# google/speedy

Measured on AMD Instinct MI355X. Metric: Msamples/s processed (16 kHz mono, 3.5x nonlinear), higher is better.
Workload: dtype int16 samples; f64 DFT, f32 features, int32 AMDF/OLA

## Files before the change

### include/speedy_hip.h

```cpp
#ifndef SPEEDY_HIP_H_
#define SPEEDY_HIP_H_
#include <stddef.h>
#include <stdint.h>
#ifdef __cplusplus
extern "C" {
#endif

#ifndef SPX_FEATURE_COUNT
#define SPX_FEATURE_COUNT 15
#endif

typedef struct spx_plan* spx_plan_t;

typedef struct {
  int64_t in_off;
  int64_t n_in;
  int64_t out_off;
  int64_t out_cap;
  int32_t channels;
  float speed;
  float nonlinear;
  float feedback;
} spx_stream_job;

typedef struct {
  float* tension;
  float* speed;
  float* features;
  float* spectrogram;
  float* normalized;
} spx_taps;

const char* spx_last_error(void);
int spx_abi_version(void);

spx_plan_t spx_plan_create(int sample_rate, int match_matlab);
void spx_plan_destroy(spx_plan_t plan);
int spx_plan_frame_step(spx_plan_t plan);
int spx_plan_window_size(spx_plan_t plan);
int spx_plan_fft_size(spx_plan_t plan);
int spx_plan_future(spx_plan_t plan);
int spx_plan_max_required(spx_plan_t plan);
int64_t spx_plan_frames(spx_plan_t plan, int64_t n_in);
int64_t spx_plan_out_capacity(spx_plan_t plan, int64_t n_in, float speed);
int64_t spx_plan_out_capacity_for(spx_plan_t plan, int64_t n_in, float speed, float nonlinear);

size_t spx_batch_workspace_bytes(spx_plan_t plan, const spx_stream_job* jobs, int n_streams);

int spx_batch_run(spx_plan_t plan, const spx_stream_job* jobs, int n_streams, const int16_t* in,
                  int16_t* out, int64_t* n_out, void* workspace, size_t workspace_bytes,
                  const spx_taps* taps, void* hip_stream);

int spx_batch_run_rate(spx_plan_t plan, const spx_stream_job* jobs, const float* rates, int n_streams, const int16_t* in,
                       int16_t* out, int64_t* n_out, void* workspace, size_t workspace_bytes,
                       const spx_taps* taps, void* hip_stream);
size_t spx_batch_workspace_bytes_rate(spx_plan_t plan, const spx_stream_job* jobs, const float* rates, int n_streams);
int64_t spx_plan_out_capacity_rate(spx_plan_t plan, int64_t n_in, float speed, float nonlinear, float rate);

size_t spx_batch_workspace_bytes_float(spx_plan_t plan, const spx_stream_job* jobs, const float* rates, int n_streams);
int spx_batch_run_float(spx_plan_t plan, const spx_stream_job* jobs, const float* rates, int n_streams, const float* in,
                        float* out, int64_t* n_out, void* workspace, size_t workspace_bytes,
                        const spx_taps* taps, void* hip_stream);
int spx_float_to_short(const float* in, int16_t* out, size_t n, int nonlinear_scale, void* hip_stream);
int spx_short_to_float(const int16_t* in, float* out, size_t n, void* hip_stream);

int spx_batch_run_ahead(spx_plan_t plan, const spx_stream_job* jobs, int n_streams, const int16_t* in,
                        int16_t* out, int64_t* n_out, void* workspace, size_t workspace_bytes,
                        const spx_taps* taps, void* hip_stream);

int spx_batch_run_overlapped(spx_plan_t plan, const spx_stream_job* jobs, int n_streams, const int16_t* in,
                             int16_t* out, int64_t* n_out, void* workspace, size_t workspace_bytes,
                             const spx_taps* taps, void* hip_stream);

int spx_batch_run_ahead_when(spx_plan_t plan, const spx_stream_job* jobs, int n_streams, const int16_t* in,
                             int16_t* out, int64_t* n_out, void* workspace, size_t workspace_bytes,
                             const spx_taps* taps, void* hip_stream, void* in_ready_event);

typedef struct spx_pipeline* spx_pipeline_t;
#define SPX_PIPELINE_DEVICE_OUT 1u
#define SPX_PIPELINE_FLOAT 2u
spx_pipeline_t spx_pipeline_create(spx_plan_t plan, const spx_stream_job* jobs, int n_streams, int depth, unsigned flags);
spx_pipeline_t spx_pipeline_create_mixed(const spx_plan_t* plans, int n_plans, const spx_stream_job* jobs, const int* plan_index,
                                         int n_streams, int depth, unsigned flags);
void spx_pipeline_destroy(spx_pipeline_t p);
int spx_pipeline_depth(spx_pipeline_t p);
size_t spx_pipeline_input_values(spx_pipeline_t p);
int16_t* spx_pipeline_host_input(spx_pipeline_t p);
int64_t spx_pipeline_submit(spx_pipeline_t p, const int16_t* in, int in_is_device);
int64_t spx_pipeline_submit_jobs(spx_pipeline_t p, const spx_stream_job* jobs, const int16_t* in, int in_is_device);
int spx_pipeline_jobs_fit(spx_pipeline_t p, const spx_stream_job* jobs);
int spx_pipeline_input_consumed(spx_pipeline_t p, int64_t ticket);
int spx_pipeline_wait(spx_pipeline_t p, int64_t ticket, const int16_t** out, const int64_t** offsets, const int64_t** counts);

float* spx_pipeline_host_input_float(spx_pipeline_t p);
int64_t spx_pipeline_submit_float(spx_pipeline_t p, const float* in, int in_is_device);
int64_t spx_pipeline_submit_jobs_float(spx_pipeline_t p, const spx_stream_job* jobs, const float* in, int in_is_device);
int spx_pipeline_wait_float(spx_pipeline_t p, int64_t ticket, const float** out, const int64_t** offsets, const int64_t** counts);

void* spx_host_alloc(size_t bytes);
void spx_host_free(void* p);

int spx_batch_analyze(spx_plan_t plan, const spx_stream_job* jobs, int n_streams, const int16_t* in,
                      void* workspace, size_t workspace_bytes, const spx_taps* taps, void* hip_stream);
int spx_batch_walk(spx_plan_t plan, const spx_stream_job* jobs, int n_streams, const int16_t* in,
                   int16_t* out, int64_t* n_out, void* workspace, size_t workspace_bytes,
                   const spx_taps* taps, void* hip_stream);

size_t spx_batch_workspace_bytes_mixed(const spx_plan_t* plans, int n_plans, const spx_stream_job* jobs,
                                       const int* plan_index, int n_streams);
int spx_batch_run_mixed(const spx_plan_t* plans, int n_plans, const spx_stream_job* jobs, const int* plan_index,
                        int n_streams, const int16_t* in, int16_t* out, int64_t* n_out, void* workspace,
                        size_t workspace_bytes, void* hip_stream);

int spx_batch_run_mixed_taps(const spx_plan_t* plans, int n_plans, const spx_stream_job* jobs, const int* plan_index,
                             int n_streams, const int16_t* in, int16_t* out, int64_t* n_out, void* workspace,
                             size_t workspace_bytes, const spx_taps* taps, void* hip_stream);
int spx_batch_run_mixed_ahead(const spx_plan_t* plans, int n_plans, const spx_stream_job* jobs, const int* plan_index,
                              int n_streams, const int16_t* in, int16_t* out, int64_t* n_out, void* workspace,
                              size_t workspace_bytes, void* hip_stream);

void spx_set_timing(int enabled);
void spx_set_pipeline_chunks(int chunks);
void spx_set_concurrent(int on);
int spx_timing_collect(double* sum_ms_analyze, double* sum_ms_walk, int* n_calls);
const char* spx_batch_kernel_names(spx_plan_t plan, int n_streams, int max_channels, int speedup_only);
const char* spx_batch_kernel_names_lean(spx_plan_t plan, int n_streams, int max_channels, int speedup_only);
int spx_debug_last_walk_form(void);
int spx_debug_kernel_vgprs(int which);
int spx_debug_walk_info(int sample_rate, int channels, int n_streams, int speedup_only, int short_jobs, int lean, int* out5);
int spx_debug_analysis_info(int sample_rate, int* out4);
int spx_debug_lane_consts(int sample_rate, void* out, double* tw, double* tw2, float* win);
int spx_debug_mode_resources(int sample_rate, int channels, int n_streams, int speedup_only, long long* out22);
long long spx_debug_fdiv_check(unsigned seed, unsigned denominators, int exp_lo, int exp_hi);
long long spx_debug_xfade_check(int n_lo, int n_hi);
long long spx_debug_arith_check(unsigned seed, unsigned threads, unsigned per_thread);
int spx_debug_select_check(const unsigned* d, int n_vectors, int p0, int n_lags, int max_period, int two_per_lane, int* lag_index,
                           unsigned* kmin);
int spx_debug_select_fold_check(const unsigned* d, int n_vectors, int p0, int n_lags, int want_max, int fresh, int* out3);
int spx_debug_log_check(unsigned first_block, unsigned end_block, unsigned long long* sums);
int spx_debug_last_call_concurrent(void);
double spx_timing_last_tension_ms(void);
double spx_timing_last_rate_ms(void);

int spx_batch_read_steps(spx_plan_t plan, const spx_stream_job* jobs, int n_streams, const void* workspace,
                         int32_t* steps, void* hip_stream);
int spx_batch_read_steps_mixed(const spx_plan_t* plans, int n_plans, const spx_stream_job* jobs, const int* plan_index,
                               int n_streams, const void* workspace, int32_t* steps, void* hip_stream);

void* spx_device_alloc(size_t bytes);
void spx_device_free(void* p);
int spx_batch_pack_outputs(const spx_stream_job* jobs, int n_streams, const int16_t* out, const int64_t* n_out,
                           int16_t* packed, int64_t* offsets, void* hip_stream);
int spx_copy_to_device(void* dst, const void* src, size_t bytes, void* hip_stream);
int spx_copy_to_host(void* dst, const void* src, size_t bytes, void* hip_stream);
int spx_stream_synchronize(void* hip_stream);

#ifdef __cplusplus
}
#endif
#endif
```

### speedy_amd/_lib.py

```python
import ctypes as C
import os
import subprocess

_HERE = os.path.dirname(os.path.abspath(__file__))
LIB_PATH = os.environ.get("SPEEDY_HIP_LIB") or os.path.join(_HERE, "lib", "libspeedy_hip.so")
_LIB = None

c_short_p = C.POINTER(C.c_short)
c_float_p = C.POINTER(C.c_float)
c_int64_p = C.POINTER(C.c_int64)


class StreamJob(C.Structure):
    _fields_ = [("in_off", C.c_int64), ("n_in", C.c_int64), ("out_off", C.c_int64), ("out_cap", C.c_int64),
                ("channels", C.c_int32), ("speed", C.c_float), ("nonlinear", C.c_float), ("feedback", C.c_float)]


class Taps(C.Structure):
    _fields_ = [("tension", C.c_void_p), ("speed", C.c_void_p), ("features", C.c_void_p),
                ("spectrogram", C.c_void_p), ("normalized", C.c_void_p)]


TENSION_FN = C.CFUNCTYPE(None, C.c_void_p, C.c_int, C.c_float)
FEATURES_FN = C.CFUNCTYPE(None, C.c_void_p, C.c_int, c_float_p)

SYMBOLS = {
    "spx_last_error": (C.c_char_p, []),
    "spx_abi_version": (C.c_int, []),
    "spx_plan_create": (C.c_void_p, [C.c_int, C.c_int]),
    "spx_plan_destroy": (None, [C.c_void_p]),
    "spx_plan_frame_step": (C.c_int, [C.c_void_p]),
    "spx_plan_window_size": (C.c_int, [C.c_void_p]),
    "spx_plan_fft_size": (C.c_int, [C.c_void_p]),
    "spx_plan_future": (C.c_int, [C.c_void_p]),
    "spx_plan_max_required": (C.c_int, [C.c_void_p]),
    "spx_plan_frames": (C.c_int64, [C.c_void_p, C.c_int64]),
    "spx_plan_out_capacity": (C.c_int64, [C.c_void_p, C.c_int64, C.c_float]),
    "spx_plan_out_capacity_for": (C.c_int64, [C.c_void_p, C.c_int64, C.c_float, C.c_float]),
    "spx_batch_workspace_bytes": (C.c_size_t, [C.c_void_p, C.POINTER(StreamJob), C.c_int]),
    "spx_batch_run": (C.c_int, [C.c_void_p, C.POINTER(StreamJob), C.c_int, C.c_void_p, C.c_void_p, C.c_void_p,
                                C.c_void_p, C.c_size_t, C.POINTER(Taps), C.c_void_p]),
    "spx_batch_run_rate": (C.c_int, [C.c_void_p, C.POINTER(StreamJob), c_float_p, C.c_int, C.c_void_p, C.c_void_p, C.c_void_p,
                                     C.c_void_p, C.c_size_t, C.POINTER(Taps), C.c_void_p]),
    "spx_batch_workspace_bytes_rate": (C.c_size_t, [C.c_void_p, C.POINTER(StreamJob), c_float_p, C.c_int]),
    "spx_plan_out_capacity_rate": (C.c_int64, [C.c_void_p, C.c_int64, C.c_float, C.c_float, C.c_float]),
    "spx_batch_workspace_bytes_float": (C.c_size_t, [C.c_void_p, C.POINTER(StreamJob), c_float_p, C.c_int]),
    "spx_batch_run_float": (C.c_int, [C.c_void_p, C.POINTER(StreamJob), c_float_p, C.c_int, C.c_void_p, C.c_void_p, C.c_void_p,
                                      C.c_void_p, C.c_size_t, C.POINTER(Taps), C.c_void_p]),
    "spx_float_to_short": (C.c_int, [C.c_void_p, C.c_void_p, C.c_size_t, C.c_int, C.c_void_p]),
    "spx_short_to_float": (C.c_int, [C.c_void_p, C.c_void_p, C.c_size_t, C.c_void_p]),
    "spx_batch_run_ahead": (C.c_int, [C.c_void_p, C.POINTER(StreamJob), C.c_int, C.c_void_p, C.c_void_p, C.c_void_p,
                                      C.c_void_p, C.c_size_t, C.POINTER(Taps), C.c_void_p]),
    "spx_batch_run_overlapped": (C.c_int, [C.c_void_p, C.POINTER(StreamJob), C.c_int, C.c_void_p, C.c_void_p, C.c_void_p,
                                           C.c_void_p, C.c_size_t, C.POINTER(Taps), C.c_void_p]),
    "spx_batch_run_ahead_when": (C.c_int, [C.c_void_p, C.POINTER(StreamJob), C.c_int, C.c_void_p, C.c_void_p, C.c_void_p,
                                           C.c_void_p, C.c_size_t, C.POINTER(Taps), C.c_void_p, C.c_void_p]),
    "spx_batch_workspace_bytes_mixed": (C.c_size_t, [C.POINTER(C.c_void_p), C.c_int, C.POINTER(StreamJob), C.POINTER(C.c_int), C.c_int]),
    "spx_batch_run_mixed": (C.c_int, [C.POINTER(C.c_void_p), C.c_int, C.POINTER(StreamJob), C.POINTER(C.c_int), C.c_int,
                                      C.c_void_p, C.c_void_p, C.c_void_p, C.c_void_p, C.c_size_t, C.c_void_p]),
    "spx_batch_run_mixed_ahead": (C.c_int, [C.POINTER(C.c_void_p), C.c_int, C.POINTER(StreamJob), C.POINTER(C.c_int), C.c_int,
                                      C.c_void_p, C.c_void_p, C.c_void_p, C.c_void_p, C.c_size_t, C.c_void_p]),
    "spx_batch_run_mixed_taps": (C.c_int, [C.POINTER(C.c_void_p), C.c_int, C.POINTER(StreamJob), C.POINTER(C.c_int), C.c_int,
                                           C.c_void_p, C.c_void_p, C.c_void_p, C.c_void_p, C.c_size_t, C.POINTER(Taps), C.c_void_p]),
    "spx_batch_read_steps": (C.c_int, [C.c_void_p, C.POINTER(StreamJob), C.c_int, C.c_void_p, C.POINTER(C.c_int32), C.c_void_p]),
    "spx_batch_read_steps_mixed": (C.c_int, [C.POINTER(C.c_void_p), C.c_int, C.POINTER(StreamJob), C.POINTER(C.c_int), C.c_int,
                                             C.c_void_p, C.POINTER(C.c_int32), C.c_void_p]),
    "spx_batch_analyze": (C.c_int, [C.c_void_p, C.POINTER(StreamJob), C.c_int, C.c_void_p, C.c_void_p,
                                    C.c_size_t, C.POINTER(Taps), C.c_void_p]),
    "spx_batch_walk": (C.c_int, [C.c_void_p, C.POINTER(StreamJob), C.c_int, C.c_void_p, C.c_void_p, C.c_void_p,
                                 C.c_void_p, C.c_size_t, C.POINTER(Taps), C.c_void_p]),
    "spx_set_timing": (None, [C.c_int]),
    "spx_set_pipeline_chunks": (None, [C.c_int]),
    "spx_set_concurrent": (None, [C.c_int]),
    "spx_timing_collect": (C.c_int, [C.POINTER(C.c_double), C.POINTER(C.c_double), C.POINTER(C.c_int)]),
    "spx_timing_last_tension_ms": (C.c_double, []),
    "spx_timing_last_rate_ms": (C.c_double, []),
    "spx_batch_kernel_names": (C.c_char_p, [C.c_void_p, C.c_int, C.c_int, C.c_int]),
    "spx_batch_kernel_names_lean": (C.c_char_p, [C.c_void_p, C.c_int, C.c_int, C.c_int]),
    "spx_debug_last_walk_form": (C.c_int, []),
    "spx_debug_kernel_vgprs": (C.c_int, [C.c_int]),
    "spx_debug_last_call_concurrent": (C.c_int, []),
    "spx_debug_fdiv_check": (C.c_longlong, [C.c_uint, C.c_uint, C.c_int, C.c_int]),
    "spx_debug_xfade_check": (C.c_longlong, [C.c_int, C.c_int]),
    "spx_debug_select_check": (C.c_int, [C.POINTER(C.c_uint), C.c_int, C.c_int, C.c_int, C.c_int, C.c_int, C.POINTER(C.c_int), C.POINTER(C.c_uint)]),
    "spx_debug_select_fold_check": (C.c_int, [C.POINTER(C.c_uint), C.c_int, C.c_int, C.c_int, C.c_int, C.c_int, C.POINTER(C.c_int)]),
    "spx_debug_arith_check": (C.c_longlong, [C.c_uint, C.c_uint, C.c_uint]),
    "spx_debug_log_check": (C.c_int, [C.c_uint, C.c_uint, C.POINTER(C.c_ulonglong)]),
    "spx_debug_walk_info": (C.c_int, [C.c_int, C.c_int, C.c_int, C.c_int, C.c_int, C.c_int, C.POINTER(C.c_int)]),
    "spx_debug_analysis_info": (C.c_int, [C.c_int, C.POINTER(C.c_int)]),
    "spx_debug_lane_consts": (C.c_int, [C.c_int, C.c_void_p, C.POINTER(C.c_double), C.POINTER(C.c_double), c_float_p]),
    "spx_debug_mode_resources": (C.c_int, [C.c_int, C.c_int, C.c_int, C.c_int, C.POINTER(C.c_longlong)]),
    "spx_pipeline_create": (C.c_void_p, [C.c_void_p, C.POINTER(StreamJob), C.c_int, C.c_int, C.c_uint]),
    "spx_pipeline_create_mixed": (C.c_void_p, [C.POINTER(C.c_void_p), C.c_int, C.POINTER(StreamJob), C.POINTER(C.c_int), C.c_int, C.c_int, C.c_uint]),
    "spx_pipeline_destroy": (None, [C.c_void_p]),
    "spx_pipeline_depth": (C.c_int, [C.c_void_p]),
    "spx_pipeline_input_values": (C.c_size_t, [C.c_void_p]),
    "spx_pipeline_host_input": (C.c_void_p, [C.c_void_p]),
    "spx_pipeline_submit": (C.c_int64, [C.c_void_p, C.c_void_p, C.c_int]),
    "spx_pipeline_submit_jobs": (C.c_int64, [C.c_void_p, C.POINTER(StreamJob), C.c_void_p, C.c_int]),
    "spx_pipeline_jobs_fit": (C.c_int, [C.c_void_p, C.POINTER(StreamJob)]),
    "spx_pipeline_input_consumed": (C.c_int, [C.c_void_p, C.c_int64]),
    "spx_pipeline_wait": (C.c_int, [C.c_void_p, C.c_int64, C.POINTER(C.c_void_p), C.POINTER(C.c_void_p), C.POINTER(C.c_void_p)]),
    "spx_pipeline_host_input_float": (C.c_void_p, [C.c_void_p]),
    "spx_pipeline_submit_float": (C.c_int64, [C.c_void_p, C.c_void_p, C.c_int]),
    "spx_pipeline_submit_jobs_float": (C.c_int64, [C.c_void_p, C.POINTER(StreamJob), C.c_void_p, C.c_int]),
    "spx_pipeline_wait_float": (C.c_int, [C.c_void_p, C.c_int64, C.POINTER(C.c_void_p), C.POINTER(C.c_void_p), C.POINTER(C.c_void_p)]),
    "spx_host_alloc": (C.c_void_p, [C.c_size_t]),
    "spx_host_free": (None, [C.c_void_p]),
    "spx_device_alloc": (C.c_void_p, [C.c_size_t]),
    "spx_device_free": (None, [C.c_void_p]),
    "spx_copy_to_device": (C.c_int, [C.c_void_p, C.c_void_p, C.c_size_t, C.c_void_p]),
    "spx_copy_to_host": (C.c_int, [C.c_void_p, C.c_void_p, C.c_size_t, C.c_void_p]),
    "spx_batch_pack_outputs": (C.c_int, [C.c_void_p, C.c_int, C.c_void_p, C.c_void_p, C.c_void_p, C.c_void_p, C.c_void_p]),
    "spx_stream_synchronize": (C.c_int, [C.c_void_p]),
    "sonicCreateStream": (C.c_void_p, [C.c_int, C.c_int]),
    "sonicDestroyStream": (None, [C.c_void_p]),
    "sonicWriteShortToStream": (C.c_int, [C.c_void_p, c_short_p, C.c_int]),
    "sonicReadShortFromStream": (C.c_int, [C.c_void_p, c_short_p, C.c_int]),
    "sonicWriteFloatToStream": (C.c_int, [C.c_void_p, c_float_p, C.c_int]),
    "sonicReadFloatFromStream": (C.c_int, [C.c_void_p, c_float_p, C.c_int]),
    "sonicSetRate": (None, [C.c_void_p, C.c_float]),
    "sonicSetSpeed": (None, [C.c_void_p, C.c_float]),
    "sonicFlushStream": (C.c_int, [C.c_void_p]),
    "sonicEnableNonlinearSpeedup": (None, [C.c_void_p, C.c_float]),
    "sonicSetDurationFeedbackStrength": (None, [C.c_void_p, C.c_float]),
    "getSonicBufferSize": (C.c_int, [C.c_void_p]),
    "sonicSpectrogramSize": (C.c_int, [C.c_void_p]),
    "sonicTensionCallback": (None, [C.c_void_p, TENSION_FN]),
    "getSonicTensionCallback": (C.c_void_p, [C.c_void_p]),
    "sonicSpeedCallback": (None, [C.c_void_p, TENSION_FN]),
    "getSonicSpeedCallback": (C.c_void_p, [C.c_void_p]),
    "sonicFeaturesCallback": (None, [C.c_void_p, FEATURES_FN]),
    "getSonicFeaturesCallback": (C.c_void_p, [C.c_void_p]),
    "sonicSpectrogramCallback": (None, [C.c_void_p, FEATURES_FN]),
    "getSonicSpectrogramCallback": (C.c_void_p, [C.c_void_p]),
    "sonicNormalizedSpectrogramCallback": (None, [C.c_void_p, FEATURES_FN]),
    "getSonicNormalizedSpectrogramCallback": (C.c_void_p, [C.c_void_p]),
    "sonicIntGetNumChannels": (C.c_int, [C.c_void_p]),
    "sonicIntGetSampleRate": (C.c_int, [C.c_void_p]),
    "sonicIntGetSpeed": (C.c_float, [C.c_void_p]),
    "sonicIntCreateStream": (C.c_void_p, [C.c_int, C.c_int]),
    "sonicIntDestroyStream": (None, [C.c_void_p]),
    "sonicIntSetSpeed": (None, [C.c_void_p, C.c_float]),
    "sonicIntSetRate": (None, [C.c_void_p, C.c_float]),
    "sonicIntWriteShortToStream": (C.c_int, [C.c_void_p, c_short_p, C.c_int]),
    "sonicIntWriteFloatToStream": (C.c_int, [C.c_void_p, c_float_p, C.c_int]),
    "sonicIntReadShortFromStream": (C.c_int, [C.c_void_p, c_short_p, C.c_int]),
    "sonicIntReadFloatFromStream": (C.c_int, [C.c_void_p, c_float_p, C.c_int]),
    "sonicIntFlushStream": (C.c_int, [C.c_void_p]),
    "sonicIntSamplesAvailable": (C.c_int, [C.c_void_p]),
    "sonicIntSetUserData": (None, [C.c_void_p, C.c_void_p]),
    "sonicIntGetUserData": (C.c_void_p, [C.c_void_p]),
    "speedyCreateStream": (C.c_void_p, [C.c_int]),
    "speedyDestroyStream": (None, [C.c_void_p]),
    "speedyInputFrameSize": (C.c_int, [C.c_void_p]),
    "speedyInputFrameStep": (C.c_int, [C.c_void_p]),
    "speedyFFTSize": (C.c_int, [C.c_void_p]),
    "speedyBinToFreq": (C.c_float, [C.c_void_p, C.c_int]),
    "speedyFreqToBin": (C.c_int, [C.c_void_p, C.c_float]),
    "speedyAddData": (None, [C.c_void_p, c_float_p, C.c_int64]),
    "speedyAddDataShort": (None, [C.c_void_p, c_short_p, C.c_int64]),
    "speedyComputeTension": (C.c_int, [C.c_void_p, C.c_int64, c_float_p]),
    "speedyComputeSpeedFromTension": (C.c_float, [C.c_float, C.c_float, C.c_float, C.c_void_p]),
    "speedyGetCurrentTime": (C.c_int64, [C.c_void_p]),
    "speedySpectrogram": (c_float_p, [C.c_void_p, c_float_p]),
    "speedyGetSpectrogram": (c_float_p, [C.c_void_p]),
    "speedyGetSpectrogramAtTime": (c_float_p, [C.c_void_p, C.c_int64]),
    "speedyGetNormalizedSpectrogram": (c_float_p, [C.c_void_p]),
    "speedyGetInternalState": (c_float_p, [C.c_void_p]),
    "speedyGetEnergyCompressed": (C.c_float, [C.c_void_p]),
    "speedyGetSpeechChanges": (C.c_float, [C.c_void_p]),
    "speedyHipHysteresisFuture": (C.c_int, [C.c_void_p]),
    "speedyHipHysteresisPast": (C.c_int, [C.c_void_p]),
    "speedyComputeSpectralDifference": (None, [C.c_void_p, c_float_p, c_float_p, C.c_int64]),
    "speedyComputeLocalEnergy": (None, [C.c_void_p, c_float_p, C.c_int64]),
    "speedySaveSpectrogramData": (None, [C.c_void_p, c_float_p, C.c_int64]),
    "speedyPreemphasisFilter": (None, [C.c_void_p, c_float_p, C.c_int]),
    "speedyEvaluateHysteresis": (C.c_float, [C.c_void_p, C.c_int64]),
    "speedyAddToHysteresisBuffer": (None, [C.c_void_p, C.c_float, C.c_int64]),
    "speedyGetInternalSpectrogram": (c_float_p, [C.c_void_p]),
    "speedyGetInternalNormalizedSpectrogram": (c_float_p, [C.c_void_p]),
    "speedyNormalizeByEnergy": (C.c_float, [c_float_p, c_float_p, C.c_int]),
    "CreateFirstOrderFilter": (C.c_void_p, [C.c_float]),
    "DesignFirstOrderLowpassFilter": (None, [C.c_void_p, C.c_float]),
    "IterateFirstOrderFilter": (C.c_float, [C.c_void_p, C.c_float]),
    "ResetFirstOrderFilter": (None, [C.c_void_p]),
    "DeleteFirstOrderFilter": (None, [C.c_void_p]),
    "speedyHipSetMatchMatlab": (None, [C.c_int]),
    "speedyHipCreateSonicStream": (C.c_void_p, [C.c_int, C.c_int, C.c_int]),
    "speedyHipSetCoalescing": (None, [C.c_int]),
    "speedyHipGetCoalescing": (C.c_int, []),
    "speedyHipCreateSonicStreamEx": (C.c_void_p, [C.c_int, C.c_int, C.c_int, C.c_int]),
    "speedyHipPoolStats": (None, [C.POINTER(C.c_ulonglong), C.POINTER(C.c_ulonglong)]),
    "sonicSamplesAvailable": (C.c_int, [C.c_void_p]),
    "speedyHipLastError": (C.c_char_p, []),
}


def build():
    subprocess.check_call(["make", "-s", "-C", os.path.join(_HERE, "csrc")])


def lib():
    global _LIB
    if _LIB is not None:
        return _LIB
    if not os.path.exists(LIB_PATH):
        raise RuntimeError(f"{LIB_PATH} is missing: run `python -c 'import __graft_entry__ as g; g.build()'` "
                           "(the product has no CPU fallback)")
    import torch
    L = C.CDLL(LIB_PATH)
    for name, (res, args) in SYMBOLS.items():
        if os.environ.get("SPEEDY_HIP_LIB") and not hasattr(L, name):
            continue
        fn = getattr(L, name)
        fn.restype = res
        fn.argtypes = args
    _LIB = L
    return L
```

### speedy_amd/csrc/spx_diag.hip

```cpp
#include "spx_engine.h"

extern "C" {
static const char* kernel_names(spx_plan_t plan, int n_streams, int max_channels, int speedup_only, bool lean);
const char* spx_batch_kernel_names(spx_plan_t plan, int n_streams, int max_channels, int speedup_only) {
  return kernel_names(plan, n_streams, max_channels, speedup_only, false);
}
const char* spx_batch_kernel_names_lean(spx_plan_t plan, int n_streams, int max_channels, int speedup_only) {
  return kernel_names(plan, n_streams, max_channels, speedup_only, true);
}
static const char* kernel_names(spx_plan_t plan, int n_streams, int max_channels, int speedup_only, bool lean) {
  static thread_local char buf[256];
  const SpxPlanDev& d = plan->dev;
  const SpxWalkConfig c = spx_walk_config(d, {.n_streams = n_streams, .max_channels = max_channels, .speedup_only = speedup_only != 0,
                                              .any_speed = speedup_only == 0, .lean = lean});
  size_t at = 0;
  auto put = [&](const SpxKernelChoice& k) {
    at += snprintf(buf + at, sizeof(buf) - at, "%s<", k.name);
    for (int i = 0; i < k.n_targs; i++) at += snprintf(buf + at, sizeof(buf) - at, i ? ", %d" : "%d", k.targs[i]);
    at += snprintf(buf + at, sizeof(buf) - at, ">");
  };
  put(spx_analysis_select(d.tile_frames, spx_analysis_ct_window(d)));
  at += snprintf(buf + at, sizeof(buf) - at, ";spx_tension_kernel;");
  put(c.kernel);
  return buf;
}

int spx_debug_last_call_concurrent(void) { return g_last_concurrent.load(std::memory_order_relaxed); }
int spx_debug_kernel_vgprs(int which) {
  if (which == 0) return spx_tension_vgprs();
  const int rate = (which == 2 || which == 4) ? 22050 : 16000;
  const SpxPlanDev* P = spx_internal_shared_plan(rate, 0);
  if (!P) return -1;
  switch (which) {
    case 1: return spx_walk_vgprs(*P, {.n_streams = 256, .max_channels = 1, .speedup_only = true}, nullptr);
    case 2: return spx_walk_vgprs(*P, {.n_streams = 256, .max_channels = 1, .speedup_only = true, .lean = true}, nullptr);
    case 3: case 4: return spx_analysis_vgprs(*P);
    case 5: return spx_walk_vgprs(*P, {.n_streams = 256, .max_channels = 2, .speedup_only = true}, nullptr);
    default: return -1;
  }
}

int spx_debug_walk_info(int sample_rate, int channels, int n_streams, int speedup_only, int short_jobs, int lean, int* out) {
  const SpxPlanDev* P = spx_internal_shared_plan(sample_rate, 0);
  if (!P || !out) return -1;
  const SpxWalkConfig c = spx_walk_config(*P, {.n_streams = n_streams, .max_channels = channels, .speedup_only = speedup_only != 0,
                                               .any_speed = speedup_only == 0, .short_jobs = short_jobs != 0, .lean = lean != 0});
  int scratch = -1;
  out[0] = spx_kernel_vgprs(c.kernel.fn, &scratch);
  out[1] = scratch;
  out[2] = (int)c.lds;
  out[3] = c.fast_kernel ? 16 * c.nwm + c.nwc : 0;
  out[4] = c.waves;
  return 0;
}
int spx_debug_analysis_info(int sample_rate, int* out) {
  const SpxPlanDev* P = spx_internal_shared_plan(sample_rate, 0);
  if (!P || !out) return -1;
  int scratch = -1;
  out[0] = spx_analysis_vgprs(*P, &scratch);
  out[1] = scratch;
  out[2] = (int)spx_analysis_lds_bytes(*P, true);
  out[3] = P->dft_waves;
  return 0;
}

void spx_set_timing(int enabled) { g_timing = enabled != 0; }
void spx_set_concurrent(int on) { g_concurrent = on != 0; }
void spx_set_pipeline_chunks(int chunks) { g_chunks_set = true; g_chunks = chunks < 1 ? 1 : (chunks > SPX_MAX_CHUNKS ? SPX_MAX_CHUNKS : chunks); }
static double g_last_tension_ms = 0.0, g_last_rate_ms = 0.0;
double spx_timing_last_tension_ms(void) { return g_last_tension_ms; }
double spx_timing_last_rate_ms(void) { return g_last_rate_ms; }
int spx_timing_collect(double* sum_ms_analyze, double* sum_ms_walk, int* n_calls) {
  std::lock_guard<std::mutex> g(g_tmu);
  double a = 0, w = 0, t = 0, r = 0;
  for (auto& ev : g_ev_pending) {
    HIPCHK(hipEventSynchronize(ev.b));
    float ms = 0;
    HIPCHK(hipEventElapsedTime(&ms, ev.a, ev.b));
    if (ev.kind == 0) a += ms; else if (ev.kind == 1) w += ms; else if (ev.kind == 3) r += ms; else t += ms;
    g_ev_free.push_back(ev.a);
    g_ev_free.push_back(ev.b);
  }
  g_ev_pending.clear();
  g_last_tension_ms = t;
  g_last_rate_ms = r;
  if (sum_ms_analyze) *sum_ms_analyze = a;
  if (sum_ms_walk) *sum_ms_walk = w;
  if (n_calls) *n_calls = g_calls_pending;
  g_calls_pending = 0;
  return 0;
}

void* spx_device_alloc(size_t bytes) {
  void* p = nullptr;
  if (hipMalloc(&p, bytes ? bytes : 1) != hipSuccess) { fail(-2, "spx_device_alloc failed"); return nullptr; }
  return p;
}
void spx_device_free(void* p) { if (p) (void)hipFree(p); }
int spx_copy_to_device(void* dst, const void* src, size_t bytes, void* hs) {
  HIPCHK(hipMemcpyAsync(dst, src, bytes, hipMemcpyHostToDevice, static_cast<hipStream_t>(hs)));
  return 0;
}
}

__global__ void __launch_bounds__(256)
spx_pack_offsets_kernel(const int64_t* __restrict__ n_out, const int* __restrict__ channels,
                        const int64_t* __restrict__ caps, int n, int64_t* __restrict__ offsets) {
  __shared__ int64_t sh[256];
  __shared__ int64_t carry;
  const int t = threadIdx.x;
  if (t == 0) carry = 0;
  __syncthreads();
  for (int i0 = 0; i0 < n; i0 += 256) {
    const int i = i0 + t;
    int64_t v = 0;
    if (i < n) {
      const int64_t k = n_out[i];
      int64_t f = (k == INT64_MIN ? 0 : (k > 0 ? k : -k));
      if (f > caps[i]) f = caps[i];
      v = f * channels[i];
    }
    sh[t] = v;
    __syncthreads();
    for (int d = 1; d < 256; d <<= 1) {
      const int64_t add = (t >= d) ? sh[t - d] : 0;
      __syncthreads();
      sh[t] += add;
      __syncthreads();
    }
    const int64_t base = carry;
    if (i < n) offsets[i] = base + sh[t] - v;
    __syncthreads();
    if (t == 255) carry = base + sh[255];
    __syncthreads();
  }
  if (t == 0) offsets[n] = carry;
}
__global__ void __launch_bounds__(256)
spx_pack_copy_kernel(const int16_t* __restrict__ out, const int64_t* __restrict__ out_offs,
                     const int64_t* __restrict__ offsets, int16_t* __restrict__ packed) {
  const int i = blockIdx.x;
  const int16_t* src = out + out_offs[i];
  int16_t* dst = packed + offsets[i];
  const int64_t cnt = offsets[i + 1] - offsets[i];
  const int64_t stride = (int64_t)gridDim.y * 256 * 8;
  for (int64_t e0 = ((int64_t)blockIdx.y * 256 + threadIdx.x); e0 < cnt; e0 += stride) {
    int16_t v[8];
#pragma unroll
    for (int u = 0; u < 8; u++) { const int64_t e = e0 + (int64_t)u * gridDim.y * 256; v[u] = (e < cnt) ? src[e] : (int16_t)0; }
#pragma unroll
    for (int u = 0; u < 8; u++) { const int64_t e = e0 + (int64_t)u * gridDim.y * 256; if (e < cnt) dst[e] = v[u]; }
  }
}

extern "C" {
int spx_batch_pack_outputs(const spx_stream_job* jobs, int n, const int16_t* out, const int64_t* n_out, int16_t* packed,
                           int64_t* offsets, void* hs) {
  if (!jobs || n <= 0 || !out || !n_out || !packed || !offsets) return fail(-1, "spx_batch_pack_outputs: bad arguments");
  hipStream_t st = static_cast<hipStream_t>(hs);
  const size_t need = (size_t)n * (2 * sizeof(int64_t) + sizeof(int));
  void* d_tab = nullptr;
  if (hipMallocAsync(&d_tab, need, st) != hipSuccess) return fail(-2, "spx_batch_pack_outputs: allocation failed");
  static thread_local SpxStage G;
  if (G.done) HIPCHK(hipEventSynchronize(G.done));
  else HIPCHK(hipEventCreateWithFlags(&G.done, hipEventDisableTiming));
  if (G.cap < need) {
    if (G.p) (void)hipHostFree(G.p);
    G.p = nullptr; G.cap = 0;
    HIPCHK(hipHostMalloc(&G.p, need * 2 + 1024, hipHostMallocDefault));
    G.cap = need * 2 + 1024;
  }
  unsigned char* h = static_cast<unsigned char*>(G.p);
  int64_t* h_off = reinterpret_cast<int64_t*>(h);
  int64_t* h_cap = h_off + n;
  int* h_ch = reinterpret_cast<int*>(h + (size_t)n * 2 * sizeof(int64_t));
  for (int i = 0; i < n; i++) { h_off[i] = jobs[i].out_off; h_cap[i] = jobs[i].out_cap; h_ch[i] = jobs[i].channels; }
  HIPCHK(hipMemcpyAsync(d_tab, h, need, hipMemcpyHostToDevice, st));
  HIPCHK(hipEventRecord(G.done, st));
  const int64_t* d_off = reinterpret_cast<const int64_t*>(d_tab);
  const int* d_ch = reinterpret_cast<const int*>(static_cast<unsigned char*>(d_tab) + (size_t)n * 2 * sizeof(int64_t));
  hipLaunchKernelGGL(spx_pack_offsets_kernel, dim3(1), dim3(256), 0, st, n_out, d_ch, d_off + n, n, offsets);
  hipLaunchKernelGGL(spx_pack_copy_kernel, dim3(n, 4), dim3(256), 0, st, out, d_off, offsets, packed);
  (void)hipFreeAsync(d_tab, st);
  HIPCHK(hipGetLastError());
  return 0;
}

int spx_copy_to_host(void* dst, const void* src, size_t bytes, void* hs) {
  HIPCHK(hipMemcpyAsync(dst, src, bytes, hipMemcpyDeviceToHost, static_cast<hipStream_t>(hs)));
  return 0;
}
int spx_stream_synchronize(void* hs) {
  HIPCHK(hipStreamSynchronize(static_cast<hipStream_t>(hs)));
  return 0;
}

}
```

### speedy_amd/csrc/spx_engine.h

```cpp
#pragma once
#include <algorithm>
#include <math.h>
#include <cmath>
#include <stdio.h>
#include <string.h>

#include <atomic>
#include <map>
#include <mutex>
#include <string>
#include <vector>

#include "../../include/speedy_hip.h"
#include "spx_internal.h"
#include "spx_jobs.h"
#include "spx_mode.h"

#ifndef M_PI
#define M_PI 3.14159265358979323846
#endif


extern thread_local std::string g_spx_err;
static inline int fail(int code, const std::string& msg) {
  g_spx_err = msg;
  return code;
}
#define HIPCHK(expr)                                                                          \
  do {                                                                                        \
    hipError_t e_ = (expr);                                                                   \
    if (e_ != hipSuccess) return fail(-2, std::string(#expr) + ": " + hipGetErrorString(e_)); \
  } while (0)

#include <dlfcn.h>
struct SpxRoctx {
  int (*push)(const char*) = nullptr;
  int (*pop)() = nullptr;
  SpxRoctx() {
    void* h = dlopen("librocprofiler-sdk-roctx.so", RTLD_LAZY | RTLD_LOCAL);
    if (!h) h = dlopen("librocprofiler-sdk-roctx.so.1", RTLD_LAZY | RTLD_LOCAL);
    if (!h) h = dlopen("libroctx64.so", RTLD_LAZY | RTLD_LOCAL);
    if (!h) h = dlopen("libroctx64.so.4", RTLD_LAZY | RTLD_LOCAL);
    if (h) {
      push = reinterpret_cast<int (*)(const char*)>(dlsym(h, "roctxRangePushA"));
      pop = reinterpret_cast<int (*)()>(dlsym(h, "roctxRangePop"));
      if (!push || !pop) { push = nullptr; pop = nullptr; }
    }
  }
};
struct SpxRange {
  static SpxRoctx& api() { static SpxRoctx a; return a; }
  explicit SpxRange(const char* name) { if (api().push) api().push(name); }
  ~SpxRange() { if (api().pop) api().pop(); }
};

#define SPX_MAX_CHUNKS 16
#define SPX_MAX_WALK_STREAMS 4
#define SPX_RING (2 * SPX_MAX_WALK_STREAMS)
struct SpxStage {
  void* p = nullptr;
  size_t cap = 0;
  hipEvent_t done = nullptr;
};
struct spx_plan {
  SpxPlanDev dev;
  int device = 0;
  int cu_count = 1;
  size_t lds_per_cu = 65536;
  std::mutex mu;
  SpxStage stage[2];
  int stage_next = 0;
  struct Trial {
    SpxModeTrial state = {-1, 0, -1};
    hipEvent_t ev[4] = {nullptr, nullptr, nullptr, nullptr};
  } trial;
  std::map<long long, SpxModeResources> res_cache;
  std::map<const void*, int> split_of;
  void* tables = nullptr;
  hipStream_t side = nullptr;
  hipStream_t side2 = nullptr;
  hipEvent_t ev_tension = nullptr;
  hipEvent_t ev_start = nullptr;
  hipEvent_t ev_chunk[SPX_MAX_CHUNKS] = {};
  hipEvent_t ev_walk[SPX_RING] = {};
  bool ev_walk_valid[SPX_RING] = {};
  void* ring_ws[SPX_RING] = {};
  hipStream_t ring_st[SPX_RING] = {};
  int ahead_calls = 0;
  hipEvent_t ev_call[2] = {nullptr, nullptr};
  const void* ahead_last_out = nullptr;
  const void* ahead_last_nout = nullptr;
  bool ev_call_valid[2] = {false, false};
  hipStream_t ev_call_st[2] = {nullptr, nullptr};
  std::vector<std::pair<const int*, int>> mixed_started;
  const int* ahead_started = nullptr;
  int ahead_n = 0;
  hipStream_t mix = nullptr;
  hipEvent_t ev_join = nullptr, ev_fork = nullptr, ev_an = nullptr;
  std::mutex mix_mu;
  SpxStage mix_stage[2];
  int mix_next = 0;
};

struct EvPair { hipEvent_t a, b; int kind; };
extern std::atomic<bool> g_timing;
extern std::atomic<int> g_last_concurrent;
extern std::atomic<int> g_concurrent;
extern std::atomic<bool> g_chunks_set;
extern std::atomic<int> g_chunks;
extern std::mutex g_tmu;
extern std::vector<EvPair> g_ev_pending;
extern std::vector<hipEvent_t> g_ev_free;
extern int g_calls_pending;
struct SpxDevGuard {
  std::mutex mu;
  hipEvent_t last = nullptr;
  hipStream_t last_stream = nullptr;
  bool valid = false;
};
extern SpxDevGuard g_guard[64];

static inline int64_t frames_for(const SpxPlanDev& d, int64_t n_in) {
  if (n_in < d.W + 1) return 0;
  return (n_in - d.W - 1) / d.B + 1;
}
spx_plan* shared_plan_full(int sample_rate, int match_matlab);

struct Layout {
  size_t off_streams, off_states, off_rec, off_scratch, off_order, off_flags, off_ready, total;
  int64_t max_tiles;
  int64_t total_frames;
};
Layout layout_for(const SpxPlanDev& d, const spx_stream_job* jobs, int n);
int dev_side_streams(int dev, hipStream_t* side, hipStream_t* side2);
int walk_stream_count();
int dev_walk_streams(int dev, hipStream_t* w, int n);
int ring_note(spx_plan* plan, hipStream_t st);
int ring_wait(spx_plan* plan, hipStream_t sa, const void* ws, hipStream_t st, bool* waited_prev);
bool ring_previous_in_flight(spx_plan* plan);
int ring_record(spx_plan* plan, hipStream_t on, void* ws, hipStream_t st, const void* out, const void* n_out, bool detached = false);
SpxModeEnv mode_env();
bool device_ours_cb(void* ctx);
struct SpxSpeedClass { int maxC; bool speedup_only, any_speed; };
SpxSpeedClass speed_class(const spx_stream_job* jobs, int n);
SpxModeWalk mode_walk(const SpxPlanDev& d, const SpxWalkAsk& ask);
void spx_launch_gate(const int* started, int n_walk, unsigned max_spins, hipStream_t st);
struct SpxForce { int concurrent; bool idle_start; int total_streams; hipEvent_t after_analysis; hipStream_t ahead_sa; const int** started_out;
                  bool no_exclusive;
};
struct SpxRateCall {
  std::vector<int64_t> walk_out_off, walk_out_cap;
  std::vector<unsigned char> no_trunc;
  std::vector<int> table;
  SpxRateJob* d_table = nullptr;
  int64_t* d_tsm_n = nullptr;
  const int16_t* tsm_base = nullptr;
  int max_blocks = 1;
};
struct SpxCallOpts {
  const SpxForce* force = nullptr;
  const SpxRateCall* rate = nullptr;
  bool ahead_req = false;
  bool overlap_req = false;
  void* in_ready = nullptr;
  bool split_part = false;
  bool sub = false;
  void* done_event = nullptr;
  bool detached = false;
};
int run_impl(spx_plan_t plan, const spx_stream_job* jobs, int n, const int16_t* in, int16_t* out, int64_t* n_out, void* ws, size_t ws_bytes,
             const spx_taps* taps, void* hs, bool do_a, bool do_w, const SpxCallOpts& opt = SpxCallOpts());
SpxJobLimits spx_job_limits(spx_plan_t plan);
int spx_check_jobs(spx_plan_t plan, const spx_stream_job* jobs, int n, bool rate_call = false, bool short_window = false);
int spx_read_steps(const SpxPlanDev& d, const spx_stream_job* jobs, int n, const void* ws, int32_t* steps, hipStream_t st);
```

### speedy_amd/csrc/spx_engine.hip

```cpp
#include "spx_engine.h"

__attribute__((constructor(101))) static void spx_default_hw_queues() {
  if (getenv("SPX_KEEP_HW_QUEUES") || getenv("GPU_MAX_HW_QUEUES")) return;
  setenv("GPU_MAX_HW_QUEUES", "8", 0);
  if (getenv("SPX_DEBUG_MODE")) fprintf(stderr, "[spx] GPU_MAX_HW_QUEUES was unset: set to 8 at load time (SPX_KEEP_HW_QUEUES=1 leaves the environment alone)\n");
}

thread_local std::string g_spx_err;

std::atomic<bool> g_timing{false};
std::atomic<int> g_last_concurrent{0};
std::atomic<int> g_concurrent{1};
std::atomic<bool> g_chunks_set{false};
std::atomic<int> g_chunks{1};
std::mutex g_tmu;
std::vector<EvPair> g_ev_pending;
std::vector<hipEvent_t> g_ev_free;
int g_calls_pending = 0;

SpxDevGuard g_guard[64];

int spx_kernel_vgprs(const void* fn, int* scratch_bytes) {
  static std::mutex mu;
  static std::map<const void*, std::pair<int, int>> cache;
  std::lock_guard<std::mutex> g(mu);
  auto it = cache.find(fn);
  if (it == cache.end()) {
    hipFuncAttributes a;
    int regs = 128, scratch = -1;
    if (hipFuncGetAttributes(&a, fn) == hipSuccess) { regs = (a.numRegs + 7) & ~7; scratch = (int)a.localSizeBytes; }
    (void)hipGetLastError();
    it = cache.emplace(fn, std::make_pair(regs, scratch)).first;
  }
  if (scratch_bytes) *scratch_bytes = it->second.second;
  return it->second.first;
}

#include <fcntl.h>
#include <sys/file.h>
#include <unistd.h>
static bool device_is_ours(int dev) {
  static std::mutex mu;
  static int state[64];
  static int lock_fd[64];
  static pid_t owner = 0;
  if (dev < 0 || dev >= 64) return false;
  std::lock_guard<std::mutex> g(mu);
  if (owner != getpid()) {
    for (int d = 0; d < 64; d++) { if (owner && state[d] > 0 && lock_fd[d] > 0) close(lock_fd[d]); state[d] = 0; lock_fd[d] = -1; }
    owner = getpid();
  }
  if (state[dev]) return state[dev] > 0;
  state[dev] = -1;
  if (getenv("SPX_SHARED_GPU")) return false;
  char bus[64] = "dev";
  if (hipDeviceGetPCIBusId(bus, (int)sizeof(bus), dev) != hipSuccess) { (void)hipGetLastError(); snprintf(bus, sizeof(bus), "ordinal%d", dev); }
  for (char* c = bus; *c; c++) if (*c == ':' || *c == '/') *c = '_';
  const char* dir = getenv("SPX_LOCK_DIR");
  if (!dir) dir = "/tmp";
  char path[256];
  snprintf(path, sizeof(path), "%s/spx_concurrent_%s.lock", dir, bus);
  int fd = open(path, O_CREAT | O_RDWR | O_CLOEXEC | O_NOFOLLOW, 0644);
  if (fd < 0) fd = open(path, O_RDONLY | O_CLOEXEC | O_NOFOLLOW);
  if (fd < 0) return false;
  if (flock(fd, LOCK_EX | LOCK_NB) != 0) { close(fd); return false; }
  state[dev] = 1;
  lock_fd[dev] = fd;
  return true;
}

extern "C" {

}
Layout layout_for(const SpxPlanDev& d, const spx_stream_job* jobs, int n) {
  Layout L;
  int64_t tf = 0;
  for (int i = 0; i < n; i++) tf += (jobs[i].nonlinear != 0.0f) ? frames_for(d, jobs[i].n_in) : 0;
  L.total_frames = tf;
  size_t o = 0;
  L.off_streams = o; o += ((sizeof(SpxStreamDev) * (size_t)n * SPX_MAX_CHUNKS + 255) & ~(size_t)255);
  L.off_states = o;  o += ((sizeof(SpxStreamState) * (size_t)n + 255) & ~(size_t)255);
  L.off_rec = o;     o += ((sizeof(SpxFrameRec) * (size_t)(tf + 1) + 255) & ~(size_t)255);
  L.off_scratch = o; o += ((sizeof(float) * 4 * (size_t)(tf + 1) + 255) & ~(size_t)255);
  const int TFr = std::min(spx_analysis_small_tile_frames(), d.tile_frames > 0 ? d.tile_frames : spx_analysis_small_tile_frames());
  L.max_tiles = tf / TFr + n + 1;
  L.off_order = o;   o += ((sizeof(int) * (size_t)L.max_tiles + 255) & ~(size_t)255);
  L.off_flags = o;   o += ((sizeof(int) * (size_t)L.max_tiles + 255) & ~(size_t)255);
  L.off_ready = o;   o += ((sizeof(int) * ((size_t)n + 1) + 255) & ~(size_t)255);
  L.total = o;
  return L;
}


static void build_streams(const SpxPlanDev& d, const spx_stream_job* jobs, int n, int nch,
                          std::vector<SpxStreamDev>& v, std::vector<int>& tiles_per_chunk, const SpxRateCall* rc = nullptr) {
  v.resize((size_t)n * nch);
  tiles_per_chunk.assign(nch, 0);
  int64_t fo = 0;
  const int TF = d.tile_frames;
  for (int i = 0; i < n; i++) {
    const spx_stream_job& j = jobs[i];
    const bool nonlinear = j.nonlinear != 0.0f;
    const int64_t Ttot = nonlinear ? frames_for(d, j.n_in) : 0;
    int64_t Tprev = 0;
    for (int c = 0; c < nch; c++) {
      int64_t n_c = j.n_in;
      if (c < nch - 1) n_c = (j.n_in * (c + 1) / nch) / d.B * d.B;
      SpxStreamDev& s = v[(size_t)c * n + i];
      s.in_off = j.in_off; s.n_in = n_c; s.out_off = j.out_off; s.out_cap = j.out_cap;
      s.channels = j.channels; s.speed = j.speed; s.nonlinear = j.nonlinear; s.feedback = j.feedback;
      const int64_t T = nonlinear ? frames_for(d, n_c) : 0;
      s.n_frames = (int32_t)T;
      s.frame_begin = (int32_t)Tprev;
      s.flags = (c == 0 ? SPX_F_INIT : 0) | (c == nch - 1 ? SPX_F_FLUSH : 0);
      if (rc) {
        s.out_off = rc->walk_out_off[i]; s.out_cap = rc->walk_out_cap[i];
        if (rc->no_trunc[i]) s.flags |= SPX_F_NO_TRUNC;
      }
      s.frame_off = fo;
      s.first_tile = tiles_per_chunk[c];
      tiles_per_chunk[c] += (int)((T - Tprev + TF - 1) / TF);
      Tprev = T;
    }
    fo += Ttot;
  }
}

static SpxTapsDev taps_of(const spx_taps* t) {
  SpxTapsDev d = {nullptr, nullptr, nullptr, nullptr, nullptr};
  if (t) { d.tension = t->tension; d.speed = t->speed; d.features = t->features;
           d.spectrogram = t->spectrogram; d.normalized = t->normalized; }
  return d;
}

__global__ void spx_gate_kernel(const int* started, int n_walk, unsigned max_spins) {
  if (threadIdx.x == 0) {
    for (unsigned i = 0; i < max_spins; i++) {
      if (__hip_atomic_load(started, __ATOMIC_RELAXED, __HIP_MEMORY_SCOPE_AGENT) >= n_walk) break;
      __builtin_amdgcn_s_sleep(8);
    }
  }
}
void spx_launch_gate(const int* started, int n_walk, unsigned max_spins, hipStream_t st) {
  hipLaunchKernelGGL(spx_gate_kernel, dim3(1), dim3(64), 0, st, started, n_walk, max_spins);
}
__global__ void __launch_bounds__(256)
spx_stage_kernel(const unsigned* __restrict__ src, unsigned* __restrict__ dst_a, unsigned n_a, unsigned* __restrict__ dst_b,
                 unsigned n_b, unsigned* __restrict__ zero_a, unsigned nz_a, unsigned* __restrict__ zero_b, unsigned nz_b,
                 const int* gate_started, int gate_n, unsigned gate_spins) {
  const unsigned stride = gridDim.x * blockDim.x, t0 = blockIdx.x * blockDim.x + threadIdx.x;
  for (unsigned i = t0; i < n_a; i += stride) dst_a[i] = src[i];
  for (unsigned i = t0; i < n_b; i += stride) dst_b[i] = src[n_a + i];
  for (unsigned i = t0; i < nz_a; i += stride) zero_a[i] = 0u;
  for (unsigned i = t0; i < nz_b; i += stride) zero_b[i] = 0u;
  if (gate_started != nullptr && t0 == 0) {
    for (unsigned i = 0; i < gate_spins; i++) {
      if (__hip_atomic_load(gate_started, __ATOMIC_RELAXED, __HIP_MEMORY_SCOPE_AGENT) >= gate_n) break;
      __builtin_amdgcn_s_sleep(8);
    }
  }
}
extern "C" {

static hipEvent_t take_event() {
  std::lock_guard<std::mutex> g(g_tmu);
  if (!g_ev_free.empty()) { hipEvent_t e = g_ev_free.back(); g_ev_free.pop_back(); return e; }
  hipEvent_t e;
  (void)hipEventCreate(&e);
  return e;
}

}
int dev_side_streams(int dev, hipStream_t* side, hipStream_t* side2) {
  static std::mutex mu;
  static hipStream_t s1[64], s2[64];
  const int d = (dev >= 0 && dev < 64) ? dev : 0;
  std::lock_guard<std::mutex> g(mu);
  if (!s1[d]) {
    if (hipStreamCreateWithFlags(&s1[d], hipStreamNonBlocking) != hipSuccess) { s1[d] = nullptr; return -1; }
    if (hipStreamCreateWithFlags(&s2[d], hipStreamNonBlocking) != hipSuccess) { (void)hipStreamDestroy(s1[d]); s1[d] = nullptr; s2[d] = nullptr; return -1; }
  }
  *side = s1[d]; *side2 = s2[d];
  return 0;
}

#ifndef SPX_WALK_STREAMS
#define SPX_WALK_STREAMS 3
#endif
int walk_stream_count() { return SPX_WALK_STREAMS; }
int dev_walk_streams(int dev, hipStream_t* w, int n) {
  static std::mutex mu;
  static hipStream_t s3[64][SPX_MAX_WALK_STREAMS];
  hipStream_t side = nullptr, side2 = nullptr;
  if (dev_side_streams(dev, &side, &side2)) return -1;
  const int d = (dev >= 0 && dev < 64) ? dev : 0;
  std::lock_guard<std::mutex> g(mu);
  w[0] = side2;
  for (int i = 1; i < n && i < SPX_MAX_WALK_STREAMS; i++) {
    if (!s3[d][i] && hipStreamCreateWithFlags(&s3[d][i], hipStreamNonBlocking) != hipSuccess) { s3[d][i] = nullptr; return -1; }
    w[i] = s3[d][i];
  }
  return 0;
}

int ring_note(spx_plan* plan, hipStream_t st) {
  const int cur = plan->ahead_calls & 1;
  if (!plan->ev_call[cur]) HIPCHK(hipEventCreateWithFlags(&plan->ev_call[cur], hipEventDisableTiming));
  HIPCHK(hipEventRecord(plan->ev_call[cur], st));
  plan->ev_call_valid[cur] = true;
  plan->ev_call_st[cur] = st;
  return 0;
}
int ring_wait(spx_plan* plan, hipStream_t sa, const void* ws, hipStream_t st, bool* waited_prev) {
  const int c = plan->ahead_calls % SPX_RING;
  if (waited_prev) *waited_prev = false;
  for (int back = SPX_RING; back >= 1; back--) {
    const int j = (c + SPX_RING - back) % SPX_RING;
    if (!plan->ev_walk_valid[j]) continue;
    if (back > SPX_RING / 2 || plan->ring_ws[j] == ws || plan->ring_st[j] != st) {
      HIPCHK(hipStreamWaitEvent(sa, plan->ev_walk[j], 0));
      if (back == 1 && waited_prev) *waited_prev = true;
    }
  }
  return 0;
}
bool ring_previous_in_flight(spx_plan* plan) {
  const int j = (plan->ahead_calls + SPX_RING - 1) % SPX_RING;
  const bool f = plan->ev_walk_valid[j] && hipEventQuery(plan->ev_walk[j]) == hipErrorNotReady;
  (void)hipGetLastError();
  return f;
}
int ring_record(spx_plan* plan, hipStream_t on, void* ws, hipStream_t st, const void* out, const void* n_out, bool detached) {
  const int c = plan->ahead_calls % SPX_RING;
  if (!plan->ev_walk[c]) HIPCHK(hipEventCreateWithFlags(&plan->ev_walk[c], hipEventDisableTiming));
  HIPCHK(hipEventRecord(plan->ev_walk[c], on));
  if (on != st && !detached) HIPCHK(hipStreamWaitEvent(st, plan->ev_walk[c], 0));
  plan->ev_walk_valid[c] = true;
  plan->ring_ws[c] = ws;
  plan->ring_st[c] = st;
  plan->ahead_last_out = out;
  plan->ahead_last_nout = n_out;
  plan->ahead_calls++;
  return 0;
}

SpxModeEnv mode_env() {
  SpxModeEnv e;
  e.concurrent_enabled = g_concurrent.load() != 0;
  e.chunks_set = g_chunks_set.load();
  e.chunks = g_chunks.load();
  return e;
}
bool device_ours_cb(void* ctx) { return device_is_ours(*static_cast<int*>(ctx)); }
SpxSpeedClass speed_class(const spx_stream_job* jobs, int n) {
  SpxSpeedClass c = {1, true, true};
  for (int i = 0; i < n; i++) {
    if (jobs[i].channels > c.maxC) c.maxC = jobs[i].channels;
    const bool ok = jobs[i].speed > 0.0f && jobs[i].speed < SPX_FAST_MAX_SPEED && jobs[i].nonlinear >= 0.0f && jobs[i].nonlinear <= 1.0f;
    if (!(ok && jobs[i].speed > 1.0f)) c.speedup_only = false;
    if (!ok) c.any_speed = false;
  }
  if (c.speedup_only) c.any_speed = false;
  return c;
}
SpxModeWalk mode_walk(const SpxPlanDev& d, const SpxWalkAsk& ask) {
  const SpxWalkConfig c = spx_walk_config(d, ask);
  SpxModeWalk w;
  w.lds = c.lds; w.waves = c.waves; w.fast_kernel = c.fast_kernel; w.nwc = c.nwc;
  w.vgprs = spx_kernel_vgprs(c.kernel.fn);
  return w;
}
static const SpxModeResources& mode_resources(spx_plan* plan, int n, int maxC, bool speedup_only, bool any_speed = false, bool short_window = false) {
  const long long key = ((long long)n << 16) ^ ((long long)maxC << 3) ^ (short_window ? 4 : 0) ^ (any_speed ? 2 : 0) ^ (speedup_only ? 1 : 0);
  auto it = plan->res_cache.find(key);
  if (it != plan->res_cache.end()) return it->second;
  const SpxPlanDev& d = plan->dev;
  SpxModeResources R;
  memset(&R, 0, sizeof(R));
  R.cu_count = plan->cu_count;
  R.lds_per_cu = plan->lds_per_cu;
  R.walk = mode_walk(d, {.n_streams = n, .max_channels = maxC, .speedup_only = speedup_only, .any_speed = any_speed, .short_window = short_window});
  R.walk_lean = R.walk;
  if (maxC == 1 && n <= plan->cu_count && R.walk.fast_kernel && R.walk.nwc > 0) {
    R.walk_lean = mode_walk(d, {.n_streams = n, .max_channels = maxC, .speedup_only = speedup_only, .any_speed = any_speed, .lean = true});
    R.lean_valid = true;
  }
  R.tension_lds = spx_tension_lds_bytes();
  R.tension_vgprs = spx_tension_vgprs();
  R.tile_default = d.tile_frames;
  R.tile_big = spx_analysis_tile_frames();
  R.tile_small = spx_analysis_small_tile_frames();
  SpxPlanDev d8 = d;
  d8.tile_frames = R.tile_small;
  R.an_lds_default = spx_analysis_lds_bytes(d, maxC == 1);
  R.an_vgprs_default = spx_analysis_vgprs(d);
  R.an_lds_small = spx_analysis_lds_bytes(d8, maxC == 1);
  R.an_vgprs_small = spx_analysis_vgprs(d8);
  if (plan->res_cache.size() > 64) plan->res_cache.clear();
  return plan->res_cache.emplace(key, R).first->second;
}
extern "C" int spx_debug_mode_resources(int sample_rate, int channels, int n_streams, int speedup_only, long long* out) {
  spx_plan* plan = shared_plan_full(sample_rate, 0);
  if (!plan || !out || n_streams < 1) return -1;
  std::lock_guard<std::mutex> g(plan->mu);
  const SpxModeResources& R = mode_resources(plan, n_streams, channels < 1 ? 1 : channels, speedup_only != 0, speedup_only == 0);
  const long long v[22] = {R.cu_count, (long long)R.lds_per_cu, (long long)R.walk.lds, R.walk.waves, R.walk.vgprs, R.walk.fast_kernel, R.walk.nwc,
                           (long long)R.walk_lean.lds, R.walk_lean.waves, R.walk_lean.vgprs, R.walk_lean.fast_kernel, R.walk_lean.nwc, R.lean_valid,
                           (long long)R.tension_lds, R.tension_vgprs, R.tile_default, R.tile_big, R.tile_small, (long long)R.an_lds_default,
                           (long long)R.an_lds_small, R.an_vgprs_default, R.an_vgprs_small};
  for (int i = 0; i < 22; i++) out[i] = v[i];
  return 0;
}

static int stage_tables(spx_plan* plan, const std::vector<SpxStreamDev>& sv, const std::vector<int>& order, SpxStreamDev* dstreams,
                        int* d_order, int* d_flags, unsigned n_flags, int* d_ready, unsigned n_ready, hipStream_t on, hipEvent_t* done,
                        const int* gate_started = nullptr, int gate_n = 0, unsigned gate_spins = 0) {
  const size_t b_sv = sizeof(SpxStreamDev) * sv.size(), b_or = sizeof(int) * order.size();
  SpxStage& G = plan->stage[plan->stage_next];
  plan->stage_next ^= 1;
  if (G.done) HIPCHK(hipEventSynchronize(G.done));
  else HIPCHK(hipEventCreateWithFlags(&G.done, hipEventDisableTiming));
  if (G.cap < b_sv + b_or) {
    if (G.p) (void)hipHostFree(G.p);
    G.p = nullptr; G.cap = 0;
    const size_t cap = (b_sv + b_or) * 2 + 4096;
    HIPCHK(hipHostMalloc(&G.p, cap, hipHostMallocDefault));
    G.cap = cap;
  }
  unsigned char* hp = static_cast<unsigned char*>(G.p);
  memcpy(hp, sv.data(), b_sv);
  if (b_or) memcpy(hp + b_sv, order.data(), b_or);
  hipLaunchKernelGGL(spx_stage_kernel, dim3(64), dim3(256), 0, on, reinterpret_cast<const unsigned*>(hp),
                     reinterpret_cast<unsigned*>(dstreams), (unsigned)(b_sv / 4), reinterpret_cast<unsigned*>(d_order), (unsigned)(b_or / 4),
                     reinterpret_cast<unsigned*>(d_flags), n_flags, reinterpret_cast<unsigned*>(d_ready), n_ready, gate_started, gate_n, gate_spins);
  HIPCHK(hipEventRecord(G.done, on));
  *done = G.done;
  return 0;
}

struct SpxTimed {
  hipEvent_t a = nullptr, b = nullptr;
  hipStream_t s = nullptr;
  int kind = 0;
  SpxTimed(bool on, int kind_, hipStream_t s_) : s(s_), kind(kind_) {
    if (on) { a = take_event(); b = take_event(); (void)hipEventRecord(a, s); }
  }
  ~SpxTimed() {
    if (!a) return;
    (void)hipEventRecord(b, s);
    std::lock_guard<std::mutex> g(g_tmu);
    g_ev_pending.push_back({a, b, kind});
  }
};

int run_impl(spx_plan_t plan, const spx_stream_job* jobs, int n, const int16_t* in, int16_t* out,
             int64_t* n_out, void* ws, size_t ws_bytes, const spx_taps* taps, void* hs, bool do_a,
             bool do_w, const SpxCallOpts& opt) {
  const SpxForce* force = opt.force;
  if (spx_check_jobs(plan, jobs, n, opt.rate != nullptr, force && force->no_exclusive)) return -1;
  SpxRange range_(do_a && do_w ? "spx_batch_run" : (do_a ? "spx_batch_analyze" : "spx_batch_walk"));
  SpxPlanDev d = plan->dev;
  Layout L = layout_for(d, jobs, n);
  if (ws_bytes < L.total || !ws) return fail(-1, "spx_batch: workspace too small");
  const SpxSpeedClass SC = speed_class(jobs, n);
  const int maxC = SC.maxC;
  const bool speedup_only = SC.speedup_only && !opt.rate, any_speed = SC.any_speed && !opt.rate;
  std::lock_guard<std::mutex> plan_lock(plan->mu);
  if (!opt.split_part) plan->split_of.erase(ws);
  const bool short_window_res = opt.force && opt.force->no_exclusive;
  const SpxModeResources& R = mode_resources(plan, n, maxC, speedup_only, any_speed, short_window_res);
  hipStream_t st = static_cast<hipStream_t>(hs);
  SpxModeShape S;
  S.n = n; S.max_channels = maxC; S.do_a = do_a; S.do_w = do_w; S.has_frames = L.total_frames > 0;
  S.forced = force != nullptr;
  S.force_concurrent = force && force->concurrent != 0;
  S.force_ahead = force && force->ahead_sa != nullptr;
  S.force_total_streams = force ? force->total_streams : n;
  S.ahead_req = opt.ahead_req; S.overlap_req = opt.overlap_req;
  SpxModeEnv E = mode_env();
  if (opt.rate) E.concurrent_enabled = false;
  SpxModeRuntime T;
  memset(&T, 0, sizeof(T));
  const int two_back = (plan->ahead_calls + SPX_RING - 2) % SPX_RING;
  T.two_workspaces = plan->ev_walk_valid[two_back] && plan->ring_ws[two_back] == ws;
  T.trial_key = ((long long)n << 40) ^ ((long long)L.total_frames << 8) ^ (maxC << 3) ^ (any_speed ? 4 : 0) ^ (speedup_only ? 2 : 0) ^ (opt.overlap_req ? 1 : 0);
  T.device_ours = device_ours_cb;
  T.device_ctx = &plan->device;
  spx_plan::Trial& TR = plan->trial;
  if (TR.state.key == T.trial_key && TR.state.choice < 0 && TR.state.calls >= 3 && TR.ev[1] && TR.ev[3] &&
      hipEventQuery(TR.ev[1]) == hipSuccess && hipEventQuery(TR.ev[3]) == hipSuccess)
    T.trial_times_ready = hipEventElapsedTime(&T.ms_seq, TR.ev[0], TR.ev[1]) == hipSuccess &&
                          hipEventElapsedTime(&T.ms_con, TR.ev[2], TR.ev[3]) == hipSuccess;
  (void)hipGetLastError();
  SpxMode M = spx_choose_mode(S, R, E, T, TR.state);
  SpxDevGuard& guard = g_guard[(plan->device >= 0 && plan->device < 64) ? plan->device : 0];
  std::unique_lock<std::mutex> guard_lock(guard.mu, std::defer_lock);
  bool idle_start = force ? force->idle_start : false;
  if (M.want_concurrent && !force) {
    guard_lock.lock();
    const hipError_t q = guard.valid ? hipEventQuery(guard.last) : hipSuccess;
    (void)hipGetLastError();
    idle_start = (q == hipSuccess);
    if (guard.valid && guard.last_stream != st && q == hipErrorNotReady) {
      T.guard_busy = true;
      M = spx_choose_mode(S, R, E, T, TR.state);
      guard_lock.unlock();
    }
  }
  static const bool dbg_trial = getenv("SPX_DEBUG_TRIAL") != nullptr;
  if (dbg_trial && TR.state.choice < 0 && M.trial_next.choice >= 0 && T.trial_times_ready)
    fprintf(stderr, "[spx trial] n=%d maxC=%d: concurrent %.3f ms, in sequence %.3f ms -> %s\n", n, maxC, T.ms_con, T.ms_seq,
            M.trial_next.choice ? "concurrent" : "sequence");
  TR.state = M.trial_next;
  d.tile_frames = M.tile_frames;
  const int nch = M.nch;
  const bool concurrent = M.concurrent, ahead = M.ahead;
  const bool chunk_ahead = M.chunk_ahead && !force;
  std::vector<SpxStreamDev> sv;
  std::vector<int> tiles;
  build_streams(d, jobs, n, nch, sv, tiles, opt.rate);
  if (opt.rate && (concurrent || ahead || chunk_ahead || !do_a || !do_w || force)) return fail(-1, "spx_batch_run_rate: internal: not a plain call in sequence");
  unsigned char* w = static_cast<unsigned char*>(ws);
  SpxStreamDev* dstreams = reinterpret_cast<SpxStreamDev*>(w + L.off_streams);
  SpxStreamState* states = reinterpret_cast<SpxStreamState*>(w + L.off_states);
  SpxFrameRec* rec = reinterpret_cast<SpxFrameRec*>(w + L.off_rec);
  float* scratch = reinterpret_cast<float*>(w + L.off_scratch);
  int* d_order = reinterpret_cast<int*>(w + L.off_order);
  int* d_flags = reinterpret_cast<int*>(w + L.off_flags);
  int* d_ready = reinterpret_cast<int*>(w + L.off_ready);
  SpxTapsDev td = taps_of(taps);
  const bool timed = g_timing.load() && do_a && do_w;
  if (do_a && do_w) g_last_concurrent.store(concurrent ? 1 : (ahead ? 2 : 0), std::memory_order_relaxed);
  static const bool dbg_mode = getenv("SPX_DEBUG_MODE") != nullptr;
  if (dbg_mode)
    fprintf(stderr, "[spx mode] rate %d n %d maxC %d: co_resident %d doubtful %d lean %d want_concurrent %d chunks %d tiles %d -> %s%s\n",
            d.rate, n, maxC, (int)M.co_resident, (int)M.doubtful, (int)M.launch_lean, (int)M.want_concurrent, nch, tiles[0],
            concurrent ? "concurrent" : (ahead ? (M.seq_ahead ? "ahead (kernels in sequence)" : "ahead") : (chunk_ahead ? "sequence, producers ahead" : "sequence")),
            M.walk2 ? ", walk kernels overlapping" : "");
  hipStream_t stw = st;
  const bool detached = opt.detached && M.walk2 && !force;
  if (do_w && !force && !detached && ring_note(plan, st)) return -2;
  if (do_w && !force && detached) { plan->ev_call_valid[plan->ahead_calls & 1] = false; plan->ev_call_st[plan->ahead_calls & 1] = nullptr; }
  if (M.walk2) {
    hipStream_t wst[SPX_MAX_WALK_STREAMS];
    const int nws = walk_stream_count();
    if (dev_walk_streams(plan->device, wst, nws)) return fail(-1, "spx_batch: no walk streams");
    const int cur = plan->ahead_calls & 1;
    stw = wst[plan->ahead_calls % nws];
    const bool same_out = !opt.sub && (out == plan->ahead_last_out || n_out == plan->ahead_last_nout);
    const bool foreign_prev = !plan->ev_call_valid[cur ^ 1] || plan->ev_call_st[cur ^ 1] != st;
    if (detached) { }
    else if (same_out || (foreign_prev && plan->ahead_calls > 0)) HIPCHK(hipStreamWaitEvent(stw, plan->ev_call[cur], 0));
    else if (plan->ev_call_valid[cur ^ 1]) HIPCHK(hipStreamWaitEvent(stw, plan->ev_call[cur ^ 1], 0));
  }
  hipStream_t sa = st;
  if (nch > 1 || concurrent || ahead) {
    if (!plan->side) {
      if (dev_side_streams(plan->device, &plan->side, &plan->side2)) return fail(-1, "spx_batch: no side streams");
      HIPCHK(hipEventCreateWithFlags(&plan->ev_start, hipEventDisableTiming));
      HIPCHK(hipEventCreateWithFlags(&plan->ev_tension, hipEventDisableTiming));
      for (auto& e : plan->ev_chunk) HIPCHK(hipEventCreateWithFlags(&e, hipEventDisableTiming));
    }
    sa = M.ahead_forced ? force->ahead_sa : plan->side;
  }
  std::vector<int> order;
  if (concurrent) {
    order.reserve((size_t)tiles[0]);
    std::vector<int> cnt(n);
    int maxT = 0;
    for (int i = 0; i < n; i++) {
      cnt[i] = (i + 1 < n ? sv[i + 1].first_tile : tiles[0]) - sv[i].first_tile;
      if (cnt[i] > maxT) maxT = cnt[i];
    }
    for (int t = 0; t < maxT; t++)
      for (int i = 0; i < n; i++)
        if (t < cnt[i]) order.push_back(sv[i].first_tile + t);
  }
  bool waited_prev = false;
  if ((ahead || chunk_ahead) && !force) {
    if (ring_wait(plan, sa, ws, st, &waited_prev)) return -2;
    if (opt.in_ready) HIPCHK(hipStreamWaitEvent(sa, static_cast<hipEvent_t>(opt.in_ready), 0));
  }
  if (!ahead && !chunk_ahead && opt.in_ready) HIPCHK(hipStreamWaitEvent(st, static_cast<hipEvent_t>(opt.in_ready), 0));
  hipEvent_t staged_ev = nullptr;
  const bool ahead_gate = ahead && !force && plan->ahead_started != nullptr && plan->ahead_n > 0 && !waited_prev &&
                          ring_previous_in_flight(plan);
  const int rc = stage_tables(plan, sv, opt.rate ? opt.rate->table : order, dstreams, opt.rate ? reinterpret_cast<int*>(opt.rate->d_table) : d_order, d_flags, concurrent ? (unsigned)tiles[0] : 0u, d_ready,
                    (concurrent || ahead) ? (unsigned)n + 1u : 0u, (ahead || chunk_ahead) ? sa : st, &staged_ev,
                    ahead_gate ? plan->ahead_started : nullptr, plan->ahead_n, 8000u);
  if (rc) return rc;
  if (M.trial_slot >= 0) {
    hipEvent_t& e0 = TR.ev[2 * M.trial_slot];
    if (!e0) HIPCHK(hipEventCreate(&e0));
    HIPCHK(hipEventRecord(e0, st));
  }
  if (sa != st && !ahead && !chunk_ahead) {
    HIPCHK(hipStreamWaitEvent(sa, staged_ev, 0));
    if (concurrent) HIPCHK(hipStreamWaitEvent(plan->side2, staged_ev, 0));
  }
  for (int c = 0; c < nch; c++) {
    SpxStreamDev* dj = dstreams + (size_t)c * n;
    if (concurrent && do_w && idle_start)
      hipLaunchKernelGGL(spx_gate_kernel, dim3(1), dim3(64), 0, sa, d_ready + n, n, 1200u);
    if (do_a && tiles[c] > 0) {
      SpxTimed tm(timed, 0, sa);
      spx_launch_analysis(d, dj, n, tiles[c], in, rec, td, concurrent ? d_order : nullptr, concurrent ? d_flags : nullptr, maxC == 1, sa);
    }
    if (force && force->after_analysis && c == nch - 1) HIPCHK(hipEventRecord(force->after_analysis, sa));
    if (sa != st) HIPCHK(hipEventRecord(plan->ev_chunk[c], sa));
    if (sa != st && !concurrent && !ahead) HIPCHK(hipStreamWaitEvent(st, plan->ev_chunk[c], 0));
    if (do_w) {
      hipStream_t stn = concurrent ? plan->side2 : (ahead ? sa : st);
      {
        SpxTimed tm(timed, 2, stn);
        spx_launch_tension(d, dj, n, states, rec, scratch, td, concurrent ? d_flags : nullptr, (concurrent || ahead) ? d_ready : nullptr, stn);
      }
      if (concurrent || ahead) HIPCHK(hipEventRecord(plan->ev_tension, stn));
      if (ahead) HIPCHK(hipStreamWaitEvent(stw, plan->ev_tension, 0));
      {
        SpxTimed tm(timed, 1, stw);
        const SpxWalkAsk ask = {.n_streams = n, .max_channels = maxC, .speedup_only = speedup_only, .any_speed = any_speed, .lean = M.launch_lean,
                                .short_window = short_window_res || (!force && M.walk2 && !M.launch_lean && maxC > 1)};
        spx_launch_walk(d, ask, dj, in, out, opt.rate ? opt.rate->d_tsm_n : n_out, states, scratch, (concurrent || ahead) ? d_ready : nullptr,
                        (M.exclusive_cu && !(force && force->no_exclusive)) ? R.lds_per_cu / 2 + 1024 : 0, stw);
      }
      if (opt.rate && c == nch - 1) {
        SpxTimed tm(timed, 3, stw);
        spx_launch_rate_batch(opt.rate->d_table, n, opt.rate->max_blocks, states, opt.rate->d_tsm_n, opt.rate->tsm_base, out, n_out, stw);
      }
      if (M.ahead_forced && force->started_out) *force->started_out = d_ready + n;
      if (c == nch - 1 && !force) {
        if (ring_record(plan, stw, ws, st, out, n_out, detached)) return -2;
        plan->ahead_started = (concurrent || ahead) ? d_ready + n : nullptr;
        plan->ahead_n = n;
        plan->mixed_started.clear();
      }
    }
    if (concurrent) {
      HIPCHK(hipStreamWaitEvent(st, plan->ev_chunk[c], 0));
      HIPCHK(hipStreamWaitEvent(st, plan->ev_tension, 0));
    }
  }
  if (concurrent && !force) {
    if (!guard.last) HIPCHK(hipEventCreateWithFlags(&guard.last, hipEventDisableTiming));
    HIPCHK(hipEventRecord(guard.last, st));
    guard.last_stream = st;
    guard.valid = true;
  }
  if (M.trial_slot >= 0) {
    hipEvent_t& e1 = TR.ev[2 * M.trial_slot + 1];
    if (!e1) HIPCHK(hipEventCreate(&e1));
    HIPCHK(hipEventRecord(e1, st));
  }
  if (opt.done_event && do_w) HIPCHK(hipEventRecord(static_cast<hipEvent_t>(opt.done_event), detached ? stw : st));
  if (timed) { std::lock_guard<std::mutex> g(g_tmu); g_calls_pending++; }
  HIPCHK(hipGetLastError());
  return 0;
}

#define SPX_SPLIT_LIMIT 4
struct SplitPlan { int k; std::vector<int> first; std::vector<size_t> ws_off, ws_bytes; size_t total; };
static SplitPlan split_geometry(const spx_plan* plan, const spx_stream_job* jobs, int n, int max_mult) {
  SplitPlan P;
  P.k = 1; P.total = 0;
  const int cu = plan->cu_count > 0 ? plan->cu_count : 1;
  if (max_mult > SPX_SPLIT_LIMIT) max_mult = SPX_SPLIT_LIMIT;
  if (n <= cu || n > max_mult * cu) return P;
  P.k = (n + cu - 1) / cu;
  size_t o = 0;
  for (int i = 0; i < P.k; i++) {
    const int a = (int)((long long)n * i / P.k), b = (int)((long long)n * (i + 1) / P.k);
    P.first.push_back(a);
    const size_t bytes = layout_for(plan->dev, jobs + a, b - a).total;
    P.ws_off.push_back(o); P.ws_bytes.push_back(bytes);
    o += (bytes + 255) & ~(size_t)255;
  }
  P.first.push_back(n);
  P.total = o;
  return P;
}
static int run_split(spx_plan_t plan, const spx_stream_job* jobs, int n, const int16_t* in, int16_t* out, int64_t* n_out, void* ws,
                     size_t ws_bytes, const spx_taps* taps, void* hs, const SpxCallOpts& opt) {
  if (!plan || !jobs || n <= 0) return fail(-1, "spx_batch: bad arguments");
  SplitPlan P = split_geometry(plan, jobs, n, opt.ahead_req && opt.overlap_req ? 2 : 1);
  if (P.k > 1 && (g_chunks_set.load() || ws_bytes < P.total)) P.k = 1;
  if (P.k > 1) {
    const SpxSpeedClass SC = speed_class(jobs, n);
    const int maxC = SC.maxC;
    std::lock_guard<std::mutex> plan_lock(plan->mu);
    const int m = P.first[1] - P.first[0];
    const SpxModeResources& R = mode_resources(plan, m, maxC, SC.speedup_only, SC.any_speed);
    SpxModeShape S;
    memset(&S, 0, sizeof(S));
    S.n = m; S.max_channels = maxC; S.do_a = S.do_w = true; S.has_frames = true; S.force_total_streams = m;
    S.ahead_req = S.overlap_req = true;
    SpxModeRuntime T;
    memset(&T, 0, sizeof(T));
    T.trial_key = -2;
    T.device_ours = device_ours_cb;
    T.device_ctx = &plan->device;
    const SpxModeTrial none = {-1, 0, -1};
    const SpxMode M = spx_choose_mode(S, R, mode_env(), T, none);
    if (!(M.ahead && M.walk2)) P.k = 1;
  }
  if (P.k <= 1) return run_impl(plan, jobs, n, in, out, n_out, ws, ws_bytes, taps, hs, true, true, opt);
  for (int i = 0; i < P.k; i++)
    if (spx_check_jobs(plan, jobs + P.first[i], P.first[i + 1] - P.first[i])) return -1;
  { std::lock_guard<std::mutex> g(plan->mu); if (plan->split_of.size() > 64) plan->split_of.clear(); plan->split_of[ws] = P.k; }
  int64_t rows = 0;
  for (int i = 0; i < P.k; i++) {
    const int a = P.first[i], m = P.first[i + 1] - a;
    spx_taps t;
    if (taps) {
      t = *taps;
      if (t.tension) t.tension += rows;
      if (t.speed) t.speed += rows;
      if (t.features) t.features += rows * SPX_FEATURE_COUNT;
      if (t.spectrogram) t.spectrogram += rows * (int64_t)plan->dev.N;
      if (t.normalized) t.normalized += rows * (int64_t)plan->dev.W;
      for (int j = a; j < a + m; j++) rows += jobs[j].nonlinear != 0.0f ? frames_for(plan->dev, jobs[j].n_in) : 0;
    }
    SpxCallOpts o;
    o.ahead_req = o.overlap_req = true;
    o.split_part = true;
    o.sub = i > 0;
    o.in_ready = opt.in_ready;
    if (i == P.k - 1) o.done_event = opt.done_event;
    const int rc = run_impl(plan, jobs + a, m, in, out, n_out + a, static_cast<unsigned char*>(ws) + P.ws_off[i], P.ws_bytes[i],
                            taps ? &t : nullptr, hs, true, true, o);
    if (rc) return rc;
  }
  return 0;
}

int spx_internal_run(spx_plan_t plan, const spx_stream_job* jobs, int n, const int16_t* in, int16_t* out, int64_t* n_out, void* ws,
                     size_t ws_bytes, const spx_taps* taps, void* hs, bool ahead, bool overlap, void* in_ready, void* done_event,
                     bool detached) {
  SpxCallOpts o;
  o.ahead_req = ahead; o.overlap_req = overlap; o.in_ready = in_ready; o.done_event = done_event; o.detached = detached;
  return run_split(plan, jobs, n, in, out, n_out, ws, ws_bytes, taps, hs, o);
}

SpxJobLimits spx_job_limits(spx_plan_t plan) { return {plan->dev.W, plan->dev.B, spx_internal_analysis_fits(plan->dev)}; }
int spx_check_jobs(spx_plan_t plan, const spx_stream_job* jobs, int n, bool rate_call, bool short_window) {
  if (!plan || !jobs || n <= 0) return fail(-1, "spx_batch: bad arguments");
  const SpxJobLimits L = spx_job_limits(plan);
  for (int i = 0; i < n; i++) {
    const SpxJobFault f = spx_check_job(L, jobs[i]);
    if (f != SPX_JOB_OK) return fail(-1, std::string("spx_batch: ") + spx_job_fault_text(f));
  }
  const SpxSpeedClass SC = speed_class(jobs, n);
  std::lock_guard<std::mutex> plan_lock(plan->mu);
  const SpxModeResources& R = mode_resources(plan, n, SC.maxC, SC.speedup_only && !rate_call, SC.any_speed && !rate_call, short_window);
  if (R.walk.lds > 160 * 1024)
    return fail(-1, "spx_batch: too many channels for the walk kernel's LDS window");
  return 0;
}

extern "C" {
size_t spx_batch_workspace_bytes(spx_plan_t plan, const spx_stream_job* jobs, int n_streams) {
  if (!plan || !jobs || n_streams < 1) return 0;
  return std::max(layout_for(plan->dev, jobs, n_streams).total, split_geometry(plan, jobs, n_streams, SPX_SPLIT_LIMIT).total);
}
int spx_batch_run(spx_plan_t plan, const spx_stream_job* jobs, int n, const int16_t* in, int16_t* out,
                  int64_t* n_out, void* ws, size_t ws_bytes, const spx_taps* taps, void* hs) {
  return run_split(plan, jobs, n, in, out, n_out, ws, ws_bytes, taps, hs, SpxCallOpts());
}
int spx_batch_run_ahead(spx_plan_t plan, const spx_stream_job* jobs, int n, const int16_t* in, int16_t* out,
                        int64_t* n_out, void* ws, size_t ws_bytes, const spx_taps* taps, void* hs) {
  return spx_internal_run(plan, jobs, n, in, out, n_out, ws, ws_bytes, taps, hs, true, false, nullptr, nullptr, false);
}
int spx_batch_run_overlapped(spx_plan_t plan, const spx_stream_job* jobs, int n, const int16_t* in, int16_t* out,
                             int64_t* n_out, void* ws, size_t ws_bytes, const spx_taps* taps, void* hs) {
  return spx_internal_run(plan, jobs, n, in, out, n_out, ws, ws_bytes, taps, hs, true, true, nullptr, nullptr, false);
}
int spx_batch_run_ahead_when(spx_plan_t plan, const spx_stream_job* jobs, int n, const int16_t* in, int16_t* out,
                             int64_t* n_out, void* ws, size_t ws_bytes, const spx_taps* taps, void* hs, void* in_ready_event) {
  return spx_internal_run(plan, jobs, n, in, out, n_out, ws, ws_bytes, taps, hs, true, false, in_ready_event, nullptr, false);
}
int spx_batch_analyze(spx_plan_t plan, const spx_stream_job* jobs, int n, const int16_t* in, void* ws,
                      size_t ws_bytes, const spx_taps* taps, void* hs) {
  return run_impl(plan, jobs, n, in, nullptr, nullptr, ws, ws_bytes, taps, hs, true, false);
}
int spx_batch_walk(spx_plan_t plan, const spx_stream_job* jobs, int n, const int16_t* in, int16_t* out,
                   int64_t* n_out, void* ws, size_t ws_bytes, const spx_taps* taps, void* hs) {
  return run_impl(plan, jobs, n, in, out, n_out, ws, ws_bytes, taps, hs, false, true);
}

}

static int rate_ratio(int sample_rate, float rate, int* old_rate, int* new_rate) {
  if (!(rate > 0.0f) || !std::isfinite(rate)) return fail(-1, "sonicSetRate: rate must be finite and > 0");
  const float q = sample_rate / rate;
  if (!(q < 2147483520.0f)) return fail(-1, "sonicSetRate: rate too small for this sample rate");
  int o = sample_rate, w = (int)q;
  while (w > (1 << 14) || o > (1 << 14)) { w >>= 1; o >>= 1; }
  if (w < 1) return fail(-1, "sonicSetRate: rate too large for this sample rate");
  if (o < 1) return fail(-1, "sonicSetRate: rate too small for this sample rate");
  *old_rate = o; *new_rate = w;
  return 0;
}
static int64_t rate_frames(int64_t m, int old_rate, int new_rate) {
  return m >= 2 ? ((m - 1) * (int64_t)new_rate + old_rate - 1) / old_rate : 0;
}
struct RateLayout { size_t off_table, off_tsm_n, off_tsm, total; std::vector<int64_t> tsm_off, tsm_cap; };
static void rate_layout(spx_plan_t plan, const spx_stream_job* jobs, const float* rates, int n, RateLayout& RL) {
  size_t o = (spx_batch_workspace_bytes(plan, jobs, n) + 255) & ~(size_t)255;
  RL.off_table = o; o += (sizeof(SpxRateJob) * (size_t)n + 255) & ~(size_t)255;
  RL.off_tsm_n = o; o += (sizeof(int64_t) * (size_t)n + 255) & ~(size_t)255;
  RL.off_tsm = o;
  RL.tsm_off.assign(n, 0); RL.tsm_cap.assign(n, 0);
  int64_t v = 0;
  for (int i = 0; i < n; i++) {
    if (rates[i] == 1.0f) continue;
    RL.tsm_off[i] = v;
    RL.tsm_cap[i] = spx_internal_out_bound(plan->dev, jobs[i].n_in, jobs[i].speed, jobs[i].nonlinear != 0.0f);
    v += (RL.tsm_cap[i] * jobs[i].channels + 7) & ~(int64_t)7;
  }
  RL.total = o + sizeof(int16_t) * (size_t)v + 128;
}
extern "C" {
int64_t spx_plan_out_capacity_rate(spx_plan_t plan, int64_t n_in, float speed, float nonlinear, float rate) {
  if (!plan) { fail(-1, "spx_plan_out_capacity_rate: bad arguments"); return -1; }
  const SpxJobFault f = spx_check_job(spx_job_limits(plan), {0, n_in, 0, 0, 1, speed, nonlinear, 0.0f});
  if (f != SPX_JOB_OK) return fail(-1, std::string("spx_batch: ") + spx_job_fault_text(f));
  const int64_t cap = spx_internal_out_bound(plan->dev, n_in, speed, nonlinear != 0.0f);
  if (rate == 1.0f) return cap;
  int o = 1, w = 1;
  if (rate_ratio(plan->dev.rate, rate, &o, &w)) return -1;
  return rate_frames(cap, o, w) + 1;
}
size_t spx_batch_workspace_bytes_rate(spx_plan_t plan, const spx_stream_job* jobs, const float* rates, int n_streams) {
  if (!rates) return spx_batch_workspace_bytes(plan, jobs, n_streams);
  if (!plan || !jobs || n_streams < 1) { fail(-1, "spx_batch: bad arguments"); return 0; }
  bool any = false;
  for (int i = 0; i < n_streams; i++) { int o, w; if (rate_ratio(plan->dev.rate, rates[i], &o, &w)) return 0; any = any || rates[i] != 1.0f; }
  if (spx_check_jobs(plan, jobs, n_streams, any)) return 0;
  RateLayout RL;
  rate_layout(plan, jobs, rates, n_streams, RL);
  return RL.total;
}
int spx_batch_run_rate(spx_plan_t plan, const spx_stream_job* jobs, const float* rates, int n, const int16_t* in, int16_t* out,
                       int64_t* n_out, void* ws, size_t ws_bytes, const spx_taps* taps, void* hs) {
  if (!plan || !jobs || n <= 0) return fail(-1, "spx_batch: bad arguments");
  bool any = false;
  std::vector<int> oldR(n, 1), newR(n, 1);
  if (rates)
    for (int i = 0; i < n; i++) {
      if (rate_ratio(plan->dev.rate, rates[i], &oldR[i], &newR[i])) return -1;
      any = any || rates[i] != 1.0f;
    }
  if (!any) return spx_batch_run(plan, jobs, n, in, out, n_out, ws, ws_bytes, taps, hs);
  if (!in || !out || !n_out || !ws || (reinterpret_cast<uintptr_t>(out) & 1)) return fail(-1, "spx_batch_run_rate: bad arguments");
  if (spx_check_jobs(plan, jobs, n, true)) return -1;
  RateLayout RL;
  rate_layout(plan, jobs, rates, n, RL);
  if (ws_bytes < RL.total) return fail(-1, "spx_batch_run_rate: workspace too small (spx_batch_workspace_bytes_rate)");
  unsigned char* w = static_cast<unsigned char*>(ws);
  SpxRateCall RC;
  RC.d_table = reinterpret_cast<SpxRateJob*>(w + RL.off_table);
  RC.d_tsm_n = reinterpret_cast<int64_t*>(w + RL.off_tsm_n);
  RC.tsm_base = reinterpret_cast<const int16_t*>(w + RL.off_tsm);
  const int64_t tsm_from_out = (int64_t)((reinterpret_cast<intptr_t>(RC.tsm_base) - reinterpret_cast<intptr_t>(out)) / (intptr_t)sizeof(int16_t));
  RC.walk_out_off.resize(n); RC.walk_out_cap.resize(n); RC.no_trunc.resize(n);
  std::vector<SpxRateJob> tab((size_t)n);
  memset(tab.data(), 0, sizeof(SpxRateJob) * (size_t)n);
  for (int i = 0; i < n; i++) {
    const bool resample = rates[i] != 1.0f;
    SpxRateJob& J = tab[i];
    J.fin_off = jobs[i].out_off; J.fin_cap = jobs[i].out_cap;
    J.channels = jobs[i].channels; J.old_rate = oldR[i]; J.new_rate = newR[i]; J.rate = rates[i];
    J.bypass = resample ? 0 : 1;
    J.tsm_off = RL.tsm_off[i]; J.tsm_cap = RL.tsm_cap[i];
    J.n_blocks = 1;
    if (resample && jobs[i].out_cap > 0) J.n_blocks = spx_rate_batch_blocks(std::min(jobs[i].out_cap, rate_frames(J.tsm_cap, J.old_rate, J.new_rate)), J.channels);
    if (J.n_blocks > RC.max_blocks) RC.max_blocks = J.n_blocks;
    RC.no_trunc[i] = resample ? 1 : 0;
    RC.walk_out_off[i] = resample ? tsm_from_out + RL.tsm_off[i] : jobs[i].out_off;
    RC.walk_out_cap[i] = resample ? RL.tsm_cap[i] : jobs[i].out_cap;
  }
  static_assert(sizeof(SpxRateJob) % sizeof(int) == 0, "the staging kernel copies 32-bit words");
  RC.table.resize(sizeof(SpxRateJob) / sizeof(int) * (size_t)n);
  memcpy(RC.table.data(), tab.data(), sizeof(SpxRateJob) * (size_t)n);
  SpxCallOpts o;
  o.rate = &RC;
  return run_impl(plan, jobs, n, in, out, n_out, ws, ws_bytes, taps, hs, true, true, o);
}
}
int spx_read_steps(const SpxPlanDev& d, const spx_stream_job* jobs, int n, const void* ws, int32_t* steps, hipStream_t st) {
  const Layout L = layout_for(d, jobs, n);
  std::vector<SpxStreamState> h((size_t)n);
  HIPCHK(hipStreamSynchronize(st));
  HIPCHK(hipMemcpy(h.data(), static_cast<const unsigned char*>(ws) + L.off_states, sizeof(SpxStreamState) * (size_t)n, hipMemcpyDeviceToHost));
  for (int i = 0; i < n; i++) steps[i] = h[i].w.steps;
  return 0;
}
extern "C" {
int spx_batch_read_steps(spx_plan_t plan, const spx_stream_job* jobs, int n, const void* ws, int32_t* steps, void* hs) {
  if (!plan || !jobs || n <= 0 || !ws || !steps) return fail(-1, "spx_batch_read_steps: bad arguments");
  int k = 1;
  { std::lock_guard<std::mutex> g(plan->mu); auto it = plan->split_of.find(ws); if (it != plan->split_of.end()) k = it->second; }
  if (k <= 1) return spx_read_steps(plan->dev, jobs, n, ws, steps, static_cast<hipStream_t>(hs));
  const SplitPlan P = split_geometry(plan, jobs, n, SPX_SPLIT_LIMIT);
  if (P.k != k) return fail(-1, "spx_batch_read_steps: the jobs are not those of the call that last ran on this workspace");
  for (int i = 0; i < P.k; i++) {
    const int a = P.first[i], m = P.first[i + 1] - a;
    const int rc = spx_read_steps(plan->dev, jobs + a, m, static_cast<const unsigned char*>(ws) + P.ws_off[i], steps + a, static_cast<hipStream_t>(hs));
    if (rc) return rc;
  }
  return 0;
}
}
```

### speedy_amd/csrc/spx_mixed.hip

```cpp
#include "spx_engine.h"

extern "C" {
__global__ void spx_scatter_nout_kernel(const int64_t* __restrict__ src, const int* __restrict__ idx, int n, int64_t* __restrict__ dst) {
  const int i = blockIdx.x * blockDim.x + threadIdx.x;
  if (i < n) dst[idx[i]] = src[i];
}
struct MixedLayout { std::vector<size_t> ws_off, ws_bytes; size_t off_nout, off_idx, total; };
static MixedLayout mixed_layout(const spx_plan_t* plans, int n_plans, const std::vector<std::vector<spx_stream_job>>& gj, int n) {
  MixedLayout M;
  size_t o = 0;
  for (int g = 0; g < n_plans; g++) {
    const size_t b = gj[g].empty() ? 0 : layout_for(plans[g]->dev, gj[g].data(), (int)gj[g].size()).total;
    M.ws_off.push_back(o); M.ws_bytes.push_back(b);
    o += (b + 255) & ~(size_t)255;
  }
  M.off_nout = o; o += ((sizeof(int64_t) * (size_t)n + 255) & ~(size_t)255);
  M.off_idx = o;  o += ((sizeof(int) * (size_t)n + 255) & ~(size_t)255);
  M.total = o;
  return M;
}
static int mixed_groups(int n_plans, const spx_stream_job* jobs, const int* plan_index, int n,
                        std::vector<std::vector<spx_stream_job>>& gj, std::vector<std::vector<int>>& gi) {
  gj.assign(n_plans, {}); gi.assign(n_plans, {});
  for (int i = 0; i < n; i++) {
    const int g = plan_index ? plan_index[i] : 0;
    if (g < 0 || g >= n_plans) return fail(-1, "spx_batch_run_mixed: plan_index out of range");
    gj[g].push_back(jobs[i]); gi[g].push_back(i);
  }
  return 0;
}
size_t spx_batch_workspace_bytes_mixed(const spx_plan_t* plans, int n_plans, const spx_stream_job* jobs, const int* plan_index,
                                       int n_streams) {
  std::vector<std::vector<spx_stream_job>> gj;
  std::vector<std::vector<int>> gi;
  if (!plans || n_plans < 1 || !jobs || n_streams < 1 || mixed_groups(n_plans, jobs, plan_index, n_streams, gj, gi)) return 0;
  return mixed_layout(plans, n_plans, gj, n_streams).total;
}
static int mixed_impl(const spx_plan_t* plans, int n_plans, const spx_stream_job* jobs, const int* plan_index, int n,
                      const int16_t* in, int16_t* out, int64_t* n_out, void* ws, size_t ws_bytes, const spx_taps* taps,
                      void* hs, bool ahead_req, void* in_ready = nullptr, void* done_event = nullptr, bool detached = false);
}
int spx_internal_run_mixed(const spx_plan_t* plans, int n_plans, const spx_stream_job* jobs, const int* plan_index, int n, const int16_t* in,
                           int16_t* out, int64_t* n_out, void* ws, size_t ws_bytes, void* hs, bool ahead, void* in_ready,
                           void* done_event, bool detached) {
  return mixed_impl(plans, n_plans, jobs, plan_index, n, in, out, n_out, ws, ws_bytes, nullptr, hs, ahead, in_ready, done_event, detached);
}
extern "C" {
int spx_batch_run_mixed(const spx_plan_t* plans, int n_plans, const spx_stream_job* jobs, const int* plan_index, int n,
                        const int16_t* in, int16_t* out, int64_t* n_out, void* ws, size_t ws_bytes, void* hs) {
  return mixed_impl(plans, n_plans, jobs, plan_index, n, in, out, n_out, ws, ws_bytes, nullptr, hs, false);
}
int spx_batch_run_mixed_taps(const spx_plan_t* plans, int n_plans, const spx_stream_job* jobs, const int* plan_index, int n,
                             const int16_t* in, int16_t* out, int64_t* n_out, void* ws, size_t ws_bytes, const spx_taps* taps,
                             void* hs) {
  return mixed_impl(plans, n_plans, jobs, plan_index, n, in, out, n_out, ws, ws_bytes, taps, hs, false);
}
int spx_batch_run_mixed_ahead(const spx_plan_t* plans, int n_plans, const spx_stream_job* jobs, const int* plan_index, int n,
                              const int16_t* in, int16_t* out, int64_t* n_out, void* ws, size_t ws_bytes, void* hs) {
  return mixed_impl(plans, n_plans, jobs, plan_index, n, in, out, n_out, ws, ws_bytes, nullptr, hs, true);
}
static int mixed_impl(const spx_plan_t* plans, int n_plans, const spx_stream_job* jobs, const int* plan_index, int n,
                      const int16_t* in, int16_t* out, int64_t* n_out, void* ws, size_t ws_bytes, const spx_taps* taps,
                      void* hs, bool ahead_req, void* in_ready, void* done_event, bool detached_req) {
  if (!plans || n_plans < 1 || n_plans > 8 || !jobs || n <= 0) return fail(-1, "spx_batch_run_mixed: bad arguments");
  SpxRange range_("spx_batch_run_mixed");
  std::vector<std::vector<spx_stream_job>> gj;
  std::vector<std::vector<int>> gi;
  int rc = mixed_groups(n_plans, jobs, plan_index, n, gj, gi);
  if (rc) return rc;
  for (int g = 0; g < n_plans; g++)
    if (!gj[g].empty() && spx_check_jobs(plans[g], gj[g].data(), (int)gj[g].size())) return -1;
  const MixedLayout M = mixed_layout(plans, n_plans, gj, n);
  if (!ws || ws_bytes < M.total) return fail(-1, "spx_batch_run_mixed: workspace too small");
  hipStream_t st = static_cast<hipStream_t>(hs);
  spx_plan* lead = plans[0];
  for (int g = 0; g < n_plans; g++) if (plans[g]->device != lead->device) return fail(-1, "spx_batch_run_mixed: plans of different devices");
  std::vector<SpxModeGroup> G;
  for (int g = 0; g < n_plans; g++) {
    if (gj[g].empty()) continue;
    const SpxPlanDev& d = plans[g]->dev;
    const SpxSpeedClass SC = speed_class(gj[g].data(), (int)gj[g].size());
    const int maxC = SC.maxC;
    bool any_nl = false;
    for (const auto& j : gj[g]) any_nl = any_nl || j.nonlinear != 0.0f;
    SpxModeGroup mg;
    mg.n = (int)gj[g].size();
    mg.walk = mode_walk(d, {.n_streams = mg.n, .max_channels = maxC, .speedup_only = SC.speedup_only, .any_speed = SC.any_speed});
    mg.any_nonlinear = any_nl;
    mg.an_lds = spx_analysis_lds_bytes(d, maxC == 1);
    mg.an_vgprs = spx_analysis_vgprs(d);
    G.push_back(mg);
  }
  const int groups = (int)G.size();
  SpxModeRuntime T;
  memset(&T, 0, sizeof(T));
  T.device_ours = device_ours_cb;
  T.device_ctx = &lead->device;
  const SpxModeEnv E = mode_env();
  SpxMixedMode MM = spx_choose_mixed_mode(G.data(), groups, n, lead->cu_count, lead->lds_per_cu, spx_tension_lds_bytes(), spx_tension_vgprs(),
                                          E, ahead_req, T);
  SpxDevGuard& guard = g_guard[(lead->device >= 0 && lead->device < 64) ? lead->device : 0];
  std::unique_lock<std::mutex> guard_lock(guard.mu, std::defer_lock);
  SpxForce force = {0, false, n, nullptr, nullptr, nullptr, false};
  if (MM.concurrent) {
    guard_lock.lock();
    const hipError_t q = guard.valid ? hipEventQuery(guard.last) : hipSuccess;
    (void)hipGetLastError();
    force.idle_start = (q == hipSuccess);
    if (guard.valid && guard.last_stream != st && q == hipErrorNotReady) {
      T.guard_busy = true;
      MM = spx_choose_mixed_mode(G.data(), groups, n, lead->cu_count, lead->lds_per_cu, spx_tension_lds_bytes(), spx_tension_vgprs(), E,
                                 ahead_req, T);
      guard_lock.unlock();
    }
  }
  const bool concurrent = MM.concurrent;
  const bool ahead = MM.ahead;
  force.concurrent = concurrent ? 1 : 0;
  const bool walk2 = spx_mixed_walk2(MM, detached_req, taps != nullptr);
  static_assert(SPX_MAX_WALK_STREAMS >= 4, "two pairs of walk streams taking turns");
  hipStream_t wst[SPX_MAX_WALK_STREAMS] = {nullptr};
  if (walk2 && dev_walk_streams(lead->device, wst, 4)) return fail(-1, "spx_batch_run_mixed: no walk streams");
  force.no_exclusive = walk2;
  std::lock_guard<std::mutex> lead_lock(lead->mix_mu);
  {
    std::lock_guard<std::mutex> ring_lock(lead->mu);
    if (ring_note(lead, st)) return -2;
  }
  if (!lead->ev_fork) HIPCHK(hipEventCreateWithFlags(&lead->ev_fork, hipEventDisableTiming));
  if (in_ready && !ahead) HIPCHK(hipStreamWaitEvent(st, static_cast<hipEvent_t>(in_ready), 0));
  HIPCHK(hipEventRecord(lead->ev_fork, st));
  unsigned char* w = static_cast<unsigned char*>(ws);
  int64_t* d_nout = reinterpret_cast<int64_t*>(w + M.off_nout);
  int* d_idx = reinterpret_cast<int*>(w + M.off_idx);
  std::vector<int> order;
  order.reserve((size_t)n);
  for (int g = 0; g < n_plans; g++) order.insert(order.end(), gi[g].begin(), gi[g].end());
  auto upload_idx = [&](hipStream_t on) -> int {
    SpxStage& G = lead->mix_stage[lead->mix_next];
    lead->mix_next ^= 1;
    if (G.done) HIPCHK(hipEventSynchronize(G.done));
    else HIPCHK(hipEventCreateWithFlags(&G.done, hipEventDisableTiming));
    if (G.cap < sizeof(int) * (size_t)n) {
      if (G.p) (void)hipHostFree(G.p);
      G.p = nullptr; G.cap = 0;
      HIPCHK(hipHostMalloc(&G.p, sizeof(int) * (size_t)n * 2 + 1024, hipHostMallocDefault));
      G.cap = sizeof(int) * (size_t)n * 2 + 1024;
    }
    memcpy(G.p, order.data(), sizeof(int) * (size_t)n);
    HIPCHK(hipMemcpyAsync(d_idx, G.p, sizeof(int) * (size_t)n, hipMemcpyHostToDevice, on));
    HIPCHK(hipEventRecord(G.done, on));
    return 0;
  };
  if (!ahead && upload_idx(st)) return -2;
  std::vector<size_t> gpos(n_plans, 0);
  { size_t pos = 0; for (int g = 0; g < n_plans; g++) { gpos[g] = pos; pos += gj[g].size(); } }
  std::vector<spx_taps> gtaps(n_plans);
  if (taps) {
    size_t rows = 0, o_spec = 0, o_norm = 0;
    for (int g = 0; g < n_plans; g++) {
      spx_taps& t = gtaps[g];
      t.tension = taps->tension ? taps->tension + rows : nullptr;
      t.speed = taps->speed ? taps->speed + rows : nullptr;
      t.features = taps->features ? taps->features + rows * SPX_FEATURE_COUNT : nullptr;
      t.spectrogram = taps->spectrogram ? taps->spectrogram + o_spec : nullptr;
      t.normalized = taps->normalized ? taps->normalized + o_norm : nullptr;
      const size_t fr = gj[g].empty() ? 0 : (size_t)layout_for(plans[g]->dev, gj[g].data(), (int)gj[g].size()).total_frames;
      rows += fr; o_spec += fr * (size_t)plans[g]->dev.N; o_norm += fr * (size_t)plans[g]->dev.W;
    }
  }
  std::vector<int> ord;
  for (int g = 0; g < n_plans; g++) if (!gj[g].empty()) ord.push_back(g);
  const bool chain_analyses = MM.chain_analyses;
  if (chain_analyses) std::stable_sort(ord.begin(), ord.end(), [&](int a, int b) { return plans[a]->dev.rate < plans[b]->dev.rate; });
  hipStream_t dev_s1 = nullptr, dev_s2 = nullptr;
  if (!concurrent && (ord.size() > 1 || ahead) && dev_side_streams(lead->device, &dev_s1, &dev_s2)) return fail(-1, "spx_batch_run_mixed: no side streams");
  std::vector<const int*> started(n_plans, nullptr);
  if (ahead) {
    std::lock_guard<std::mutex> ring_lock(lead->mu);
    bool waited_prev = false;
    if (ring_wait(lead, dev_s1, ws, st, &waited_prev)) return -2;
    const bool in_flight = !waited_prev && ring_previous_in_flight(lead);
    if (in_ready) HIPCHK(hipStreamWaitEvent(dev_s1, static_cast<hipEvent_t>(in_ready), 0));
    if (upload_idx(dev_s1)) return -2;
    if (in_flight)
      for (const auto& sn : lead->mixed_started)
        if (sn.first && sn.second > 0) spx_launch_gate(sn.first, sn.second, 8000u, dev_s1);
  }
  hipEvent_t prev_an = nullptr;
  int launch_idx = 0;
  hipStream_t end_stream = nullptr;
  for (int g : ord) {
    spx_plan* p = plans[g];
    hipStream_t gs = nullptr;
    if (walk2 && launch_idx < 2) gs = wst[2 * launch_idx + (int)(lead->ahead_calls & 1)];
    else if (!concurrent && launch_idx == 0) gs = st;
    else if (!concurrent && launch_idx == 1) gs = dev_s2;
    else {
      if (!p->mix) HIPCHK(hipStreamCreateWithFlags(&p->mix, hipStreamNonBlocking));
      gs = p->mix;
    }
    launch_idx++;
    if (!p->ev_join) HIPCHK(hipEventCreateWithFlags(&p->ev_join, hipEventDisableTiming));
    if (!p->ev_an) HIPCHK(hipEventCreateWithFlags(&p->ev_an, hipEventDisableTiming));
    const bool on_walk_stream = walk2 && launch_idx <= 2;
    if (gs != st && !on_walk_stream) HIPCHK(hipStreamWaitEvent(gs, lead->ev_fork, 0));
    if (!end_stream) end_stream = gs;
    SpxForce f = force;
    if (ahead) {
      f.ahead_sa = dev_s1;
      f.started_out = &started[g];
    } else if (chain_analyses) {
      if (prev_an) HIPCHK(hipStreamWaitEvent(gs, prev_an, 0));
      f.after_analysis = p->ev_an;
      prev_an = p->ev_an;
    }
    SpxCallOpts go;
    go.force = &f;
    rc = run_impl(p, gj[g].data(), (int)gj[g].size(), in, out, d_nout + gpos[g], w + M.ws_off[g], M.ws_bytes[g], taps ? &gtaps[g] : nullptr, gs,
                  true, true, go);
    const std::string err = rc ? g_spx_err : std::string();
    hipStream_t join_to = walk2 ? end_stream : st;
    if (gs != join_to && (hipEventRecord(p->ev_join, gs) != hipSuccess || hipStreamWaitEvent(join_to, p->ev_join, 0) != hipSuccess)) {
      (void)hipGetLastError();
      (void)hipStreamSynchronize(gs);
      if (!rc) return fail(-2, "spx_batch_run_mixed: joining a group's stream failed");
    }
    if (rc) return fail(rc, err);
  }
  hipStream_t fin = (walk2 && end_stream) ? end_stream : st;
  hipLaunchKernelGGL(spx_scatter_nout_kernel, dim3((n + 255) / 256), dim3(256), 0, fin, d_nout, d_idx, n, n_out);
  if (done_event) HIPCHK(hipEventRecord(static_cast<hipEvent_t>(done_event), fin));
  {
    std::lock_guard<std::mutex> ring_lock(lead->mu);
    if (ring_record(lead, fin, ws, st, out, n_out, walk2)) return -2;
    lead->ahead_started = nullptr;
    lead->ahead_n = 0;
    lead->mixed_started.clear();
    if (ahead)
      for (int g = 0; g < n_plans; g++)
        if (started[g]) lead->mixed_started.emplace_back(started[g], (int)gj[g].size());
  }
  if (concurrent) {
    if (!guard.last) HIPCHK(hipEventCreateWithFlags(&guard.last, hipEventDisableTiming));
    HIPCHK(hipEventRecord(guard.last, st));
    guard.last_stream = st;
    guard.valid = true;
  }
  HIPCHK(hipGetLastError());
  return 0;
}

int spx_batch_read_steps_mixed(const spx_plan_t* plans, int n_plans, const spx_stream_job* jobs, const int* plan_index, int n,
                               const void* ws, int32_t* steps, void* hs) {
  if (!plans || n_plans < 1 || n_plans > 8 || !jobs || n <= 0 || !ws || !steps) return fail(-1, "spx_batch_read_steps_mixed: bad arguments");
  std::vector<std::vector<spx_stream_job>> gj;
  std::vector<std::vector<int>> gi;
  int rc = mixed_groups(n_plans, jobs, plan_index, n, gj, gi);
  if (rc) return rc;
  const MixedLayout M = mixed_layout(plans, n_plans, gj, n);
  for (int g = 0; g < n_plans; g++) {
    if (gj[g].empty()) continue;
    std::vector<int32_t> sg(gj[g].size());
    rc = spx_read_steps(plans[g]->dev, gj[g].data(), (int)gj[g].size(), static_cast<const unsigned char*>(ws) + M.ws_off[g], sg.data(),
                    static_cast<hipStream_t>(hs));
    if (rc) return rc;
    for (size_t k = 0; k < sg.size(); k++) steps[gi[g][k]] = sg[k];
  }
  return 0;
}

}
```

### speedy_amd/csrc/spx_mode.h

```cpp
#ifndef SPX_MODE_H_
#define SPX_MODE_H_
#include <stddef.h>

#define SPX_MODE_MAX_CHUNKS 16

struct SpxModeWalk {
  size_t lds;
  int waves;
  int vgprs;
  bool fast_kernel;
  int nwc;
};
struct SpxModeResources {
  int cu_count;
  size_t lds_per_cu;
  SpxModeWalk walk;
  SpxModeWalk walk_lean;
  bool lean_valid;
  size_t tension_lds;
  int tension_vgprs;
  int tile_default, tile_big, tile_small;
  size_t an_lds_default, an_lds_small;
  int an_vgprs_default, an_vgprs_small;
};
struct SpxModeShape {
  int n, max_channels;
  bool do_a, do_w;
  bool has_frames;
  bool forced;
  bool force_concurrent, force_ahead;
  int force_total_streams;
  bool ahead_req;
  bool overlap_req;
};
struct SpxModeEnv {
  bool concurrent_enabled;
  bool chunks_set;
  int chunks;
};
struct SpxModeTrial {
  long long key;
  int calls;
  int choice;
};
struct SpxModeRuntime {
  bool two_workspaces;
  bool guard_busy;
  bool trial_times_ready;
  float ms_seq, ms_con;
  long long trial_key;
  bool (*device_ours)(void*);
  void* device_ctx;
};
struct SpxMode {
  bool lean_walk;
  bool launch_lean;
  int tile_frames;
  bool co_resident, doubtful;
  int trial_slot;
  bool want_concurrent;
  bool concurrent;
  bool ahead, seq_ahead, ahead_forced;
  bool walk2;
  bool chunk_ahead;
  int nch;
  bool exclusive_cu;
  bool asked_device;
  SpxModeTrial trial_next;
};

static inline bool spx_mode_fits2(const SpxModeResources& R, const SpxModeWalk& w, size_t lds_usable) {
  return w.lds + R.tension_lds + 2 * R.an_lds_default <= lds_usable &&
         ((w.waves + 3) / 4) * w.vgprs + R.tension_vgprs + 2 * R.an_vgprs_default <= 512;
}

static inline int spx_mode_an_waves(const SpxModeResources& R, const SpxModeWalk& w) {
  const int left = 512 - ((w.waves + 3) / 4) * w.vgprs - R.tension_vgprs;
  return (left > 0 && R.an_vgprs_default > 0) ? left / R.an_vgprs_default : 0;
}

static inline SpxMode spx_mode_pass(const SpxModeShape& S, const SpxModeResources& R, const SpxModeEnv& E, const SpxModeRuntime& T,
                                    const SpxModeTrial& trial_in, bool lean_walk) {
  SpxMode M;
  M.lean_walk = lean_walk;
  M.asked_device = false;
  M.trial_next = trial_in;
  const SpxModeWalk& W = lean_walk ? R.walk_lean : R.walk;
  const bool both = S.do_a && S.do_w;
  const size_t lds_usable = R.lds_per_cu > 6144 ? R.lds_per_cu - 6144 : R.lds_per_cu;
  const size_t per_stream_lds = W.lds + R.tension_lds;
  const size_t per_stream_waves = (size_t)W.waves + 4;
  auto ours = [&]() { M.asked_device = true; return T.device_ours ? T.device_ours(T.device_ctx) : true; };
  int tile = R.tile_default;
  if (per_stream_lds + 2 * R.an_lds_default > lds_usable && both && R.tile_default == R.tile_big &&
      per_stream_lds + 2 * R.an_lds_small <= lds_usable)
    tile = R.tile_small;
  const size_t an_lds = tile == R.tile_default ? R.an_lds_default : R.an_lds_small;
  const int an_vgprs = tile == R.tile_default ? R.an_vgprs_default : R.an_vgprs_small;
  bool co_resident = false, doubtful = false;
  if (an_lds < R.lds_per_cu) {
    const size_t lds_closing = R.lds_per_cu - an_lds + 1;
    const size_t closed = ((size_t)S.n * per_stream_lds) / lds_closing + ((size_t)S.n * per_stream_waves) / 29;
    co_resident = closed < (size_t)R.cu_count && S.n <= R.cu_count;
    if (per_stream_lds + 2 * an_lds > lds_usable) co_resident = false;
    if (co_resident) {
      const int walk_regs = ((W.waves + 3) / 4) * W.vgprs;
      if (walk_regs + R.tension_vgprs + 2 * an_vgprs > 512) {
        if (walk_regs + R.tension_vgprs + an_vgprs > 512) co_resident = false;
        else doubtful = true;
      }
    }
  }
  M.doubtful = doubtful;
  int trial_slot = -1;
  if (co_resident && doubtful && both && E.concurrent_enabled && !S.forced) {
    SpxModeTrial& N = M.trial_next;
    if (N.key != T.trial_key) { N.key = T.trial_key; N.calls = 0; N.choice = -1; }
    if (N.choice < 0 && N.calls >= 3 && T.trial_times_ready) N.choice = T.ms_con < T.ms_seq ? 1 : 0;
    if (N.choice >= 0) co_resident = N.choice == 1;
    else if (N.calls == 0) { }
    else if (N.calls == 1) trial_slot = 1;
    else if (N.calls == 2) { trial_slot = 0; co_resident = false; }
    else co_resident = false;
    N.calls++;
  }
  M.co_resident = co_resident;
  M.trial_slot = trial_slot;
  bool want_concurrent = E.concurrent_enabled && co_resident && both;
  if (want_concurrent && !S.forced && !ours()) want_concurrent = false;
  if (S.forced) want_concurrent = S.force_concurrent && both;
  M.ahead_forced = S.forced && S.force_ahead && both;
  const bool chunks_free = !E.chunks_set || E.chunks == 1;
  bool seq_ahead = false;
  if (S.ahead_req && !want_concurrent && !S.forced && both && S.n <= R.cu_count && E.concurrent_enabled &&
      trial_slot < 0 && chunks_free && !lean_walk) {
    const size_t walk_lds = W.lds > R.lds_per_cu / 2 + 1024 ? W.lds : R.lds_per_cu / 2 + 1024;
    const int walk_regs = ((W.waves + 3) / 4) * W.vgprs;
    seq_ahead = walk_lds + R.tension_lds + R.an_lds_default <= lds_usable &&
                walk_regs + R.tension_vgprs + R.an_vgprs_default <= 512 && ours();
  }
  M.seq_ahead = seq_ahead;
  M.ahead = M.ahead_forced || seq_ahead ||
            (S.ahead_req && want_concurrent && !doubtful && !S.forced && trial_slot < 0 && chunks_free);
  if (!S.has_frames && !M.ahead_forced) { M.ahead = false; seq_ahead = false; M.seq_ahead = false; }
  if (M.ahead) want_concurrent = false;
  if (want_concurrent && !S.forced && T.guard_busy) want_concurrent = false;
  M.want_concurrent = want_concurrent;
  if (!want_concurrent && (!M.ahead || seq_ahead)) tile = R.tile_default;
  M.tile_frames = tile;
  int nch = both ? E.chunks : 1;
  if (both && !E.chunks_set && !want_concurrent && S.n > 2 * R.cu_count) nch = 2;
  if (M.ahead) nch = 1;
  if (nch < 1) nch = 1;
  if (nch > SPX_MODE_MAX_CHUNKS) nch = SPX_MODE_MAX_CHUNKS;
  M.nch = nch;
  M.concurrent = want_concurrent && nch == 1 && S.has_frames;
  M.walk2 = S.overlap_req && M.ahead && !S.forced && !seq_ahead;
  const int total = S.forced ? S.force_total_streams : S.n;
  M.exclusive_cu = !M.concurrent && (!M.ahead || M.ahead_forced || seq_ahead) && nch == 1 && total <= R.cu_count;
  M.launch_lean = lean_walk && (M.concurrent || M.ahead);
  M.chunk_ahead = S.ahead_req && !S.forced && both && !M.ahead && !want_concurrent && nch >= 2 && S.n > 2 * R.cu_count &&
                  E.concurrent_enabled && trial_slot < 0 && ours();
  return M;
}

static inline SpxMode spx_choose_mode(const SpxModeShape& S, const SpxModeResources& R, const SpxModeEnv& E, const SpxModeRuntime& T,
                                      const SpxModeTrial& trial_in) {
  const size_t lds_usable = R.lds_per_cu > 6144 ? R.lds_per_cu - 6144 : R.lds_per_cu;
  const bool lean_possible = S.do_a && S.do_w && S.max_channels == 1 && S.n <= R.cu_count && R.walk.fast_kernel && R.walk.nwc > 0 &&
                             !S.forced && R.lean_valid && R.walk_lean.fast_kernel && R.walk_lean.nwc == 0;
  const bool lean_fits = lean_possible && spx_mode_fits2(R, R.walk_lean, lds_usable);
  const bool lean_analysis_build = R.tile_default == R.tile_big && R.an_vgprs_default < R.an_vgprs_small;
  const bool need_lean = lean_fits && (!spx_mode_fits2(R, R.walk, lds_usable) ||
                                       (lean_analysis_build && spx_mode_an_waves(R, R.walk_lean) > spx_mode_an_waves(R, R.walk)));
  SpxMode M = spx_mode_pass(S, R, E, T, trial_in, need_lean);
  if (!need_lean && lean_fits && M.walk2 && S.overlap_req && !T.two_workspaces) {
    SpxMode L = spx_mode_pass(S, R, E, T, trial_in, true);
    L.asked_device = L.asked_device || M.asked_device;
    if (L.ahead && L.walk2) return L;
  }
  return M;
}

struct SpxModeGroup {
  int n;
  SpxModeWalk walk;
  bool any_nonlinear;
  size_t an_lds;
  int an_vgprs;
};
struct SpxMixedMode {
  bool concurrent;
  bool ahead;
  bool chain_analyses;
  bool asked_device;
};
static inline SpxMixedMode spx_choose_mixed_mode(const SpxModeGroup* G, int groups, int n_total, int cu_count, size_t lds_per_cu,
                                                 size_t tension_lds, int tension_vgprs, const SpxModeEnv& E, bool ahead_req,
                                                 const SpxModeRuntime& T) {
  SpxMixedMode M = {false, false, false, false};
  size_t cons_lds = 0, cons_waves = 0, max_ps_lds = 0, max_an_lds = 0;
  int max_walk_regs = 0, max_an_regs = 0;
  for (int g = 0; g < groups; g++) {
    const size_t ps = G[g].walk.lds + tension_lds;
    cons_lds += (size_t)G[g].n * ps;
    cons_waves += (size_t)G[g].n * (G[g].walk.waves + 4);
    if (ps > max_ps_lds) max_ps_lds = ps;
    if (G[g].any_nonlinear) {
      if (G[g].an_lds > max_an_lds) max_an_lds = G[g].an_lds;
      if (G[g].an_vgprs > max_an_regs) max_an_regs = G[g].an_vgprs;
    }
    const int wr = ((G[g].walk.waves + 3) / 4) * G[g].walk.vgprs;
    if (wr > max_walk_regs) max_walk_regs = wr;
  }
  auto ours = [&]() { M.asked_device = true; return T.device_ours ? T.device_ours(T.device_ctx) : true; };
  bool concurrent = false;
  if (max_an_lds > 0 && max_an_lds < lds_per_cu && n_total <= cu_count) {
    const size_t closed = cons_lds / (lds_per_cu - max_an_lds + 1) + cons_waves / 29;
    concurrent = closed < (size_t)cu_count;
    const size_t lds_usable = lds_per_cu > 6144 ? lds_per_cu - 6144 : lds_per_cu;
    if (max_ps_lds + 2 * max_an_lds > lds_usable) concurrent = false;
    if (max_walk_regs + tension_vgprs + 2 * max_an_regs > 512) concurrent = false;
  }
  if (!E.concurrent_enabled || groups == 0) concurrent = false;
  if (concurrent && !ours()) concurrent = false;
  if (concurrent && T.guard_busy) concurrent = false;
  M.ahead = ahead_req && !concurrent && E.concurrent_enabled && groups > 0 && n_total <= cu_count && ours();
  M.concurrent = concurrent;
  M.chain_analyses = !concurrent && groups > 1;
  return M;
}

static inline bool spx_mixed_walk2(const SpxMixedMode& M, bool detached, bool taps) {
  return M.ahead && !M.concurrent && detached && !taps;
}

#endif
```

### speedy_amd/csrc/spx_mode_table.cpp

```cpp
#include <string.h>

#include "spx_jobs.h"
#include "spx_mode.h"

#define SPX_Q_FIELDS(X)                                                                                                         \
  X(n) X(max_channels) X(do_a) X(do_w) X(has_frames) X(forced) X(force_concurrent) X(force_ahead) X(force_total_streams)        \
  X(ahead_req) X(overlap_req) X(cu_count) X(lds_per_cu) X(walk_lds) X(walk_waves) X(walk_vgprs) X(walk_fast) X(walk_nwc)        \
  X(lean_lds) X(lean_waves) X(lean_vgprs) X(lean_fast) X(lean_nwc) X(lean_valid) X(tension_lds) X(tension_vgprs)                \
  X(tile_default) X(tile_big) X(tile_small) X(an_lds_default) X(an_lds_small) X(an_vgprs_default) X(an_vgprs_small)             \
  X(concurrent_enabled) X(chunks_set) X(chunks) X(trial_state_key) X(trial_calls) X(trial_choice) X(two_workspaces)            \
  X(guard_busy) X(trial_times_ready) X(us_seq) X(us_con) X(trial_key) X(device_ours)
#define SPX_A_FIELDS(X)                                                                                                         \
  X(lean_walk) X(launch_lean) X(tile_frames) X(co_resident) X(doubtful) X(trial_slot) X(want_concurrent) X(concurrent)          \
  X(ahead) X(seq_ahead) X(ahead_forced) X(walk2) X(nch) X(exclusive_cu) X(asked_device) X(next_key) X(next_calls) X(next_choice)

enum {
#define X(f) Q_##f,
  SPX_Q_FIELDS(X)
#undef X
  Q_COUNT
};
enum {
#define X(f) A_##f,
  SPX_A_FIELDS(X)
#undef X
  A_COUNT
};

static bool ours_cb(void* ctx) { return *static_cast<long long*>(ctx) != 0; }

extern "C" {
const char* spx_mode_table_query_fields(void) {
  return
#define X(f) #f " "
      SPX_Q_FIELDS(X)
#undef X
      ;
}
const char* spx_mode_table_answer_fields(void) {
  return
#define X(f) #f " "
      SPX_A_FIELDS(X)
#undef X
      ;
}
int spx_mode_table_eval(const long long* q, int nq, long long* a, int na) {
  if (nq != Q_COUNT || na != A_COUNT) return -1;
  SpxModeShape S;
  SpxModeResources R;
  SpxModeEnv E;
  SpxModeRuntime T;
  memset(&S, 0, sizeof(S)); memset(&R, 0, sizeof(R)); memset(&E, 0, sizeof(E)); memset(&T, 0, sizeof(T));
  S.n = (int)q[Q_n]; S.max_channels = (int)q[Q_max_channels]; S.do_a = q[Q_do_a]; S.do_w = q[Q_do_w]; S.has_frames = q[Q_has_frames];
  S.forced = q[Q_forced]; S.force_concurrent = q[Q_force_concurrent]; S.force_ahead = q[Q_force_ahead];
  S.force_total_streams = (int)q[Q_force_total_streams]; S.ahead_req = q[Q_ahead_req]; S.overlap_req = q[Q_overlap_req];
  R.cu_count = (int)q[Q_cu_count]; R.lds_per_cu = (size_t)q[Q_lds_per_cu];
  R.walk = {(size_t)q[Q_walk_lds], (int)q[Q_walk_waves], (int)q[Q_walk_vgprs], q[Q_walk_fast] != 0, (int)q[Q_walk_nwc]};
  R.walk_lean = {(size_t)q[Q_lean_lds], (int)q[Q_lean_waves], (int)q[Q_lean_vgprs], q[Q_lean_fast] != 0, (int)q[Q_lean_nwc]};
  R.lean_valid = q[Q_lean_valid];
  R.tension_lds = (size_t)q[Q_tension_lds]; R.tension_vgprs = (int)q[Q_tension_vgprs];
  R.tile_default = (int)q[Q_tile_default]; R.tile_big = (int)q[Q_tile_big]; R.tile_small = (int)q[Q_tile_small];
  R.an_lds_default = (size_t)q[Q_an_lds_default]; R.an_lds_small = (size_t)q[Q_an_lds_small];
  R.an_vgprs_default = (int)q[Q_an_vgprs_default]; R.an_vgprs_small = (int)q[Q_an_vgprs_small];
  E.concurrent_enabled = q[Q_concurrent_enabled]; E.chunks_set = q[Q_chunks_set]; E.chunks = (int)q[Q_chunks];
  const SpxModeTrial trial = {q[Q_trial_state_key], (int)q[Q_trial_calls], (int)q[Q_trial_choice]};
  T.two_workspaces = q[Q_two_workspaces]; T.guard_busy = q[Q_guard_busy]; T.trial_times_ready = q[Q_trial_times_ready];
  T.ms_seq = (float)q[Q_us_seq] / 1000.0f; T.ms_con = (float)q[Q_us_con] / 1000.0f; T.trial_key = q[Q_trial_key];
  long long ours = q[Q_device_ours];
  T.device_ours = ours_cb; T.device_ctx = &ours;
  const SpxMode M = spx_choose_mode(S, R, E, T, trial);
  a[A_lean_walk] = M.lean_walk; a[A_launch_lean] = M.launch_lean; a[A_tile_frames] = M.tile_frames; a[A_co_resident] = M.co_resident;
  a[A_doubtful] = M.doubtful; a[A_trial_slot] = M.trial_slot; a[A_want_concurrent] = M.want_concurrent; a[A_concurrent] = M.concurrent;
  a[A_ahead] = M.ahead; a[A_seq_ahead] = M.seq_ahead; a[A_ahead_forced] = M.ahead_forced; a[A_walk2] = M.walk2; a[A_nch] = M.nch;
  a[A_exclusive_cu] = M.exclusive_cu; a[A_asked_device] = M.asked_device; a[A_next_key] = M.trial_next.key;
  a[A_next_calls] = M.trial_next.calls; a[A_next_choice] = M.trial_next.choice;
  return 0;
}
int spx_mode_table_mixed_mode(const long long* groups, int n_groups, int n_total, int cu_count, long long lds_per_cu, long long tension_lds,
                              int tension_vgprs, int concurrent_enabled, int ahead_req, int guard_busy, int device_ours, long long* out4) {
  SpxModeGroup G[8];
  if (n_groups < 0 || n_groups > 8) return -1;
  for (int g = 0; g < n_groups; g++) {
    const long long* p = groups + 7 * g;
    G[g].n = (int)p[0];
    G[g].walk = {(size_t)p[1], (int)p[2], (int)p[3], true, 4};
    G[g].any_nonlinear = p[4] != 0;
    G[g].an_lds = (size_t)p[5];
    G[g].an_vgprs = (int)p[6];
  }
  SpxModeEnv E;
  memset(&E, 0, sizeof(E));
  E.concurrent_enabled = concurrent_enabled; E.chunks = 1;
  SpxModeRuntime T;
  memset(&T, 0, sizeof(T));
  long long ours = device_ours;
  T.guard_busy = guard_busy; T.device_ours = ours_cb; T.device_ctx = &ours;
  const SpxMixedMode M = spx_choose_mixed_mode(G, n_groups, n_total, cu_count, (size_t)lds_per_cu, (size_t)tension_lds, tension_vgprs, E,
                                               ahead_req != 0, T);
  out4[0] = M.concurrent; out4[1] = M.ahead; out4[2] = M.chain_analyses; out4[3] = M.asked_device;
  return 0;
}
int spx_mode_table_mixed_walk2(int concurrent, int ahead, int detached, int taps) {
  SpxMixedMode M = {concurrent != 0, ahead != 0, false, false};
  return spx_mixed_walk2(M, detached != 0, taps != 0) ? 1 : 0;
}
int spx_mode_table_check_job(int W, int B, int analysis_fits, int channels, long long n_in, long long in_off, long long out_off,
                             long long out_cap, float speed, float nonlinear, float feedback) {
  const spx_stream_job j = {in_off, n_in, out_off, out_cap, channels, speed, nonlinear, feedback};
  return spx_check_job({W, B, analysis_fits != 0}, j);
}
const char* spx_mode_table_job_fault_text(int code) {
  return code < SPX_JOB_OK || code > SPX_JOB_TOO_LONG ? "" : spx_job_fault_text(static_cast<SpxJobFault>(code));
}
}
```

### speedy_amd/csrc/spx_plan.hip

```cpp
#include "spx_engine.h"
#include "spx_twiddle.h"
#include "spx_twiddle_hashes.h"

int64_t spx_internal_out_bound(const SpxPlanDev& P, int64_t n_in, float speed, bool nonlinear) {
  const int64_t slack = 4 * (int64_t)P.maxRequired + 1024;
  if (speed >= 1.0f) return n_in + slack;
  double s = nonlinear ? 0.01 : (double)speed;
  if (s < 1e-4) s = 1e-4;
  return (int64_t)((double)(n_in + 2 * (int64_t)P.maxRequired) * (2.0 / s)) + slack;
}

void spx_lane_consts_fill(const double* tw, const double* tw2, const float* win, unsigned char* out) {
  double* d = reinterpret_cast<double*>(out);
  auto put = [&](int c, int lane, const double* src, int idx) {
    d[2 * (64 * c + lane)] = src[2 * idx];
    d[2 * (64 * c + lane) + 1] = src[2 * idx + 1];
  };
  for (int lane = 0; lane < 64; lane++) {
    const int bb = lane < 60 ? lane : 0;
    for (int j = 1; j < 4; j++) {
      put(SPX_LC_W1 + j - 1, lane, tw, bb * j);
      put(SPX_LC_W2 + j - 1, lane, tw, 4 * (bb >> 2) * j);
    }
    for (int u = 0; u < 2; u++) {
      const int b3 = lane + 64 * u, p3 = (b3 < 80) ? (b3 >> 4) : 0;
      put(SPX_LC_W3 + 2 * u, lane, tw, 16 * p3);
      put(SPX_LC_W3 + 2 * u + 1, lane, tw, 32 * p3);
    }
    for (int u = 0; u < 4; u++) {
      const int k = lane + 64 * u;
      put(SPX_LC_WU + u, lane, tw2, k < 240 ? k : 0);
    }
    float* f = reinterpret_cast<float*>(out + 16 * (size_t)(64 * SPX_LC_WN + lane));
    const int wi[4] = {2 * bb, 2 * bb + 1, 2 * bb + 120, 2 * bb + 121};
    for (int k = 0; k < 4; k++) f[k] = win[wi[k]] * SPX_WIN_SCALE;
  }
}
static void plan_host_tables(int W, double* tw, double* tw2, float* win) {
  for (int t = 0; t < W; t++) {
    spx_tw::entry(t, W, &tw[2 * t]);
    spx_tw::entry(t, 2L * W, &tw2[2 * t]);
    double c = 1.0, sn = 0.0;
    if (W > 1) spx_tw::sincos_2pi(t, W - 1, &c, &sn);
    win[t] = 0.54 - 0.46 * c;
  }
}

void spx_internal_set_error(const char* msg) { g_spx_err = msg ? msg : ""; }
extern "C" {

const char* spx_last_error(void) { return g_spx_err.c_str(); }
void spx_debug_twiddle_entry(long k, long n, double* c, double* s) { spx_tw::sincos_2pi(k, n, c, s); }
unsigned long long spx_debug_twiddle_hash(long den, long count) {
  uint64_t h = 0xcbf29ce484222325ull;
  for (long t = 0; t < count; t++) {
    double e[2];
    spx_tw::entry(t, den, e);
    const unsigned char* b = reinterpret_cast<const unsigned char*>(e);
    for (int i = 0; i < 16; i++) { h ^= b[i]; h *= 0x100000001b3ull; }
  }
  return h;
}
int spx_abi_version(void) { return 1; }
int spx_debug_lane_consts(int sample_rate, void* out, double* tw, double* tw2, float* win) {
  if (!out || !tw || !tw2 || !win) return -1;
  if ((int)(1.5 * sample_rate / (float)100.0) != 240) return 0;
  plan_host_tables(240, tw, tw2, win);
  spx_lane_consts_fill(tw, tw2, win, static_cast<unsigned char*>(out));
  return SPX_LC_BYTES;
}

static int factor_radices(int n, int* radix) {
  int ns = 0;
  while (n % 4 == 0) { radix[ns++] = 4; n /= 4; }
  while (n % 2 == 0) { radix[ns++] = 2; n /= 2; }
  while (n % 3 == 0) { radix[ns++] = 3; n /= 3; }
  while (n % 5 == 0) { radix[ns++] = 5; n /= 5; }
  for (int p = 7; n > 1; p += 2)
    while (n % p == 0) { radix[ns++] = p; n /= p; }
  return ns;
}

spx_plan_t spx_plan_create(int sample_rate, int match_matlab) {
  if (sample_rate < 1000 || sample_rate > 127999) {
    fail(-1, "spx_plan_create: unsupported sample rate");
    return nullptr;
  }
  spx_plan* p = new spx_plan();
  SpxPlanDev& d = p->dev;
  memset(&d, 0, sizeof(d));
  {
    hipDeviceProp_t prop;
    if (hipGetDevice(&p->device) == hipSuccess && hipGetDeviceProperties(&prop, p->device) == hipSuccess) {
      p->cu_count = prop.multiProcessorCount > 0 ? prop.multiProcessorCount : 1;
      p->lds_per_cu = prop.maxSharedMemoryPerMultiProcessor ? (size_t)prop.maxSharedMemoryPerMultiProcessor : 65536;
    }
  }
  d.rate = sample_rate;
  d.B = (int)(sample_rate / 100.0);
  d.W = (int)(1.5 * sample_rate / (float)100.0);
  d.N = 2 * d.W;
  d.F = match_matlab ? 8 : 12;
  d.Pp = match_matlab ? 12 : 8;
  d.nstages = (d.W > 1) ? factor_radices(d.W, d.radix) : 0;
  if (d.nstages > SPX_MAX_STAGES) {
    delete p;
    fail(-1, "spx_plan_create: too many DFT stages");
    return nullptr;
  }
  d.minPeriod = sample_rate / 400;
  d.maxPeriod = sample_rate / 65;
  d.maxRequired = 2 * d.maxPeriod;
  d.skip = sample_rate > 4000 ? sample_rate / 4000 : 1;
  d.alpha = (float)exp(-1.0 / (float)100.0);
  d.one_minus_alpha = 1 - d.alpha;

  const int W = d.W;
  const int M = W - 1;
  bool rader = W > 64;
  for (int q = 2; rader && (long)q * q <= W; q++) if (W % q == 0) rader = false;
  if (rader) {
    int m = M;
    for (int q = 2; q <= 13; q++) while (m % q == 0) m /= q;
    rader = (m == 1);
  }
  if (rader) {
    d.rader = 1;
    d.nstagesM = factor_radices(M, d.radixM);
  }
  d.dft_waves = 4;
  d.tile_frames = spx_analysis_tile_frames();
  const int cand[5][2] = {{spx_analysis_tile_frames(), 4}, {spx_analysis_small_tile_frames(), 4}, {spx_analysis_small_tile_frames(), 2},
                          {spx_analysis_tiny_tile_frames(), 2}, {spx_analysis_tiny_tile_frames(), 1}};
  for (int c = 0; c < 5; c++) {
    d.tile_frames = cand[c][0];
    d.dft_waves = cand[c][1];
    if (spx_analysis_lds_bytes(d, false) <= 160 * 1024) break;
  }
  if (spx_analysis_prefers_small_tile(d)) {
    d.tile_frames = spx_analysis_small_tile_frames();
    d.dft_waves = 4;
  }
  const size_t n_tw = 2 * (size_t)W, n_win = (size_t)W, n_tf = d.F + 1, n_tp = d.Pp + 1;
  const size_t n_rd = rader ? 2 * (size_t)M : 0;
  const size_t n_ri = rader ? (size_t)M : 0;
  const size_t n_ql = rader ? (size_t)W : 0;
  const size_t bytes0 = sizeof(double) * (2 * n_tw + 2 * n_rd) + sizeof(float) * (n_win + n_tf + n_tp + 8) +
                        sizeof(int) * (2 * n_ri + n_ql);
  const bool lane_tab = !rader && W == 240;
  const size_t off_lc = (bytes0 + 15) & ~(size_t)15;
  const size_t bytes = lane_tab ? off_lc + SPX_LC_BYTES : bytes0;
  std::vector<unsigned char> host(bytes, 0);
  double* tw = reinterpret_cast<double*>(host.data());
  double* tw2 = tw + n_tw;
  double* twM = tw2 + n_tw;
  double* bfft = twM + n_rd;
  float* win = reinterpret_cast<float*>(bfft + n_rd);
  float* tf = win + n_win;
  float* tp = tf + n_tf;
  int* perm = reinterpret_cast<int*>(tp + n_tp + 8);
  int* iperm = perm + n_ri;
  int* qlog = iperm + n_ri;
  plan_host_tables(W, tw, tw2, win);
  if (lane_tab) spx_lane_consts_fill(tw, tw2, win, host.data() + off_lc);
  if (rader) {
    for (int t = 0; t < M; t++) spx_tw::entry(t, M, &twM[2 * t]);
    int g = 2;
    for (; g < W; g++) {
      long v = 1;
      int k = 0;
      do { v = (v * g) % W; k++; } while (v != 1);
      if (k == M) break;
    }
    long v = 1;
    for (int k = 0; k < M; k++) { perm[k] = (int)v; v = (v * g) % W; }
    for (int q = 0; q < M; q++) iperm[q] = perm[(M - q) % M];
    for (int q = 0; q < M; q++) qlog[iperm[q]] = q;
    std::vector<double> b(2 * (size_t)M);
    for (int q = 0; q < M; q++) { b[2 * q] = tw[2 * iperm[q]]; b[2 * q + 1] = tw[2 * iperm[q] + 1]; }
    spx_host_dft(M, d.radixM, d.nstagesM, twM, b.data(), bfft);
  }
  {
    const struct { long den, count; const double* t; } built[3] = {{W, W, tw}, {2L * W, W, tw2}, {rader ? M : 0, rader ? M : 0, twM}};
    for (const auto& b : built)
      for (const auto& pin : spx_twiddle_pins)
        if (b.count > 0 && pin.den == b.den && pin.count == b.count && spx_tw::fnv1a(b.t, 16 * (size_t)b.count) != pin.hash) {
          delete p;
          fail(-1, "spx_plan_create: a twiddle table does not hash to its pinned value (spx_twiddle_hashes.h) -- host code built with fast-math or fp contraction?");
          return nullptr;
        }
  }
  for (int i = 0; i <= d.F; i++) tf[i] = (d.F - i) / (float)d.F;
  for (int i = 0; i <= d.Pp; i++) tp[i] = (d.Pp - i) / (float)d.Pp;
  {
    hipStream_t w[SPX_MAX_WALK_STREAMS];
    (void)dev_walk_streams(p->device, w, walk_stream_count());
    (void)hipGetLastError();
  }
  if (hipMalloc(&p->tables, bytes) != hipSuccess ||
      hipMemcpy(p->tables, host.data(), bytes, hipMemcpyHostToDevice) != hipSuccess) {
    fail(-2, "spx_plan_create: device allocation/copy failed (is a GPU visible?)");
    if (p->tables) (void)hipFree(p->tables);
    delete p;
    return nullptr;
  }
  unsigned char* base = static_cast<unsigned char*>(p->tables);
  d.tw = reinterpret_cast<const double*>(base);
  d.tw2 = d.tw + n_tw;
  d.twM = d.tw2 + n_tw;
  d.bfft = d.twM + n_rd;
  d.window = reinterpret_cast<const float*>(d.bfft + n_rd);
  d.taperF = d.window + n_win;
  d.taperP = d.taperF + n_tf;
  d.perm = reinterpret_cast<const int*>(d.taperP + n_tp + 8);
  d.iperm = d.perm + n_ri;
  d.qlog = d.iperm + n_ri;
  d.lane_consts = lane_tab ? base + off_lc : nullptr;
  return p;
}

void spx_plan_destroy(spx_plan_t plan) {
  if (!plan) return;
  if (plan->side) (void)hipStreamSynchronize(plan->side);
  if (plan->side2) (void)hipStreamSynchronize(plan->side2);
  if (plan->mix) { (void)hipStreamSynchronize(plan->mix); (void)hipStreamDestroy(plan->mix); }
  if (plan->ev_join) (void)hipEventDestroy(plan->ev_join);
  if (plan->ev_an) (void)hipEventDestroy(plan->ev_an);
  if (plan->ev_fork) (void)hipEventDestroy(plan->ev_fork);
  for (auto& g : plan->mix_stage) {
    if (g.done) { (void)hipEventSynchronize(g.done); (void)hipEventDestroy(g.done); }
    if (g.p) (void)hipHostFree(g.p);
  }
  if (plan->ev_tension) (void)hipEventDestroy(plan->ev_tension);
  if (plan->ev_start) (void)hipEventDestroy(plan->ev_start);
  for (auto& e : plan->ev_chunk) if (e) (void)hipEventDestroy(e);
  for (auto& e : plan->trial.ev) if (e) (void)hipEventDestroy(e);
  for (auto& e : plan->ev_walk) if (e) { (void)hipEventSynchronize(e); (void)hipEventDestroy(e); }
  for (auto& e : plan->ev_call) if (e) (void)hipEventDestroy(e);
  for (auto& g : plan->stage) {
    if (g.done) { (void)hipEventSynchronize(g.done); (void)hipEventDestroy(g.done); }
    if (g.p) (void)hipHostFree(g.p);
  }
  if (plan->tables) (void)hipFree(plan->tables);
  delete plan;
}
int spx_plan_frame_step(spx_plan_t p) { return p->dev.B; }
int spx_plan_window_size(spx_plan_t p) { return p->dev.W; }
int spx_plan_fft_size(spx_plan_t p) { return p->dev.N; }
int spx_plan_future(spx_plan_t p) { return p->dev.F; }
int spx_plan_max_required(spx_plan_t p) { return p->dev.maxRequired; }

int64_t spx_plan_frames(spx_plan_t p, int64_t n_in) { return frames_for(p->dev, n_in); }

int64_t spx_plan_out_capacity_for(spx_plan_t p, int64_t n_in, float speed, float nonlinear) {
  return spx_internal_out_bound(p->dev, n_in, speed, nonlinear != 0.0f);
}
int64_t spx_plan_out_capacity(spx_plan_t p, int64_t n_in, float speed) {
  return spx_internal_out_bound(p->dev, n_in, speed, true);
}

}
bool spx_internal_analysis_fits(const SpxPlanDev& d) { return spx_analysis_lds_bytes(d, false) <= 160 * 1024; }

spx_plan* shared_plan_full(int sample_rate, int match_matlab) {
  static std::mutex mu;
  static std::map<std::pair<int, std::pair<int, int>>, spx_plan*> cache;
  std::lock_guard<std::mutex> g(mu);
  int dev = 0;
  (void)hipGetDevice(&dev);
  auto key = std::make_pair(dev, std::make_pair(sample_rate, match_matlab ? 1 : 0));
  auto it = cache.find(key);
  if (it != cache.end()) return it->second;
  spx_plan* p = spx_plan_create(sample_rate, match_matlab);
  if (!p) return nullptr;
  cache[key] = p;
  return p;
}
const SpxPlanDev* spx_internal_shared_plan(int sample_rate, int match_matlab) {
  spx_plan* p = shared_plan_full(sample_rate, match_matlab);
  return p ? &p->dev : nullptr;
}
int64_t spx_internal_frames_for(const SpxPlanDev& d, int64_t n_in) { return frames_for(d, n_in); }
```

Measured before the change: 49820.

## Track gate state per ring slot and optionally run tension on walk stream

Replaces the single ahead_started pointer with per-ring-slot started pointers, so the cross-call gate spin only fires when the previous call's slot is valid, in flight and uses a different workspace. It also adds a device counter for gate timeouts. A compile-time option, off by default, moves the tension kernel onto the walk stream so the event handoff is skipped. With that option off, the main runtime effect is a tighter gate condition plus an extra atomic in the timeout path.

```diff
diff --git a/include/speedy_hip.h b/include/speedy_hip.h
--- a/include/speedy_hip.h
+++ b/include/speedy_hip.h
@@ -139,6 +139,9 @@
 int spx_debug_select_fold_check(const unsigned* d, int n_vectors, int p0, int n_lags, int want_max, int fresh, int* out3);
 int spx_debug_log_check(unsigned first_block, unsigned end_block, unsigned long long* sums);
 int spx_debug_last_call_concurrent(void);
+int spx_debug_last_tension_stream(void);
+int spx_debug_tension_on_walk_enabled(void);
+long long spx_debug_gate_timeouts(spx_plan_t plan);
 double spx_timing_last_tension_ms(void);
 double spx_timing_last_rate_ms(void);
 
diff --git a/speedy_amd/_lib.py b/speedy_amd/_lib.py
--- a/speedy_amd/_lib.py
+++ b/speedy_amd/_lib.py
@@ -80,6 +80,9 @@
     "spx_debug_last_walk_form": (C.c_int, []),
     "spx_debug_kernel_vgprs": (C.c_int, [C.c_int]),
     "spx_debug_last_call_concurrent": (C.c_int, []),
+    "spx_debug_last_tension_stream": (C.c_int, []),
+    "spx_debug_tension_on_walk_enabled": (C.c_int, []),
+    "spx_debug_gate_timeouts": (C.c_longlong, [C.c_void_p]),
     "spx_debug_fdiv_check": (C.c_longlong, [C.c_uint, C.c_uint, C.c_int, C.c_int]),
     "spx_debug_xfade_check": (C.c_longlong, [C.c_int, C.c_int]),
     "spx_debug_select_check": (C.c_int, [C.POINTER(C.c_uint), C.c_int, C.c_int, C.c_int, C.c_int, C.c_int, C.POINTER(C.c_int), C.POINTER(C.c_uint)]),
diff --git a/speedy_amd/csrc/spx_diag.hip b/speedy_amd/csrc/spx_diag.hip
--- a/speedy_amd/csrc/spx_diag.hip
+++ b/speedy_amd/csrc/spx_diag.hip
@@ -26,6 +26,19 @@
 }
 
 int spx_debug_last_call_concurrent(void) { return g_last_concurrent.load(std::memory_order_relaxed); }
+int spx_debug_last_tension_stream(void) { return g_last_tension_stream.load(std::memory_order_relaxed); }
+long long spx_debug_gate_timeouts(spx_plan_t plan) {
+  if (!plan) { fail(-1, "spx_debug_gate_timeouts: bad arguments"); return -1; }
+  std::lock_guard<std::mutex> g(plan->mu);
+  if (!plan->d_gate_timeouts) return 0;
+  unsigned v = 0;
+  if (hipMemcpy(&v, plan->d_gate_timeouts, sizeof(v), hipMemcpyDeviceToHost) != hipSuccess) {
+    (void)hipGetLastError();
+    fail(-2, "spx_debug_gate_timeouts: the copy failed");
+    return -1;
+  }
+  return (long long)v;
+}
 int spx_debug_kernel_vgprs(int which) {
   if (which == 0) return spx_tension_vgprs();
   const int rate = (which == 2 || which == 4) ? 22050 : 16000;
diff --git a/speedy_amd/csrc/spx_engine.h b/speedy_amd/csrc/spx_engine.h
--- a/speedy_amd/csrc/spx_engine.h
+++ b/speedy_amd/csrc/spx_engine.h
@@ -92,9 +92,10 @@
   const void* ahead_last_nout = nullptr;
   bool ev_call_valid[2] = {false, false};
   hipStream_t ev_call_st[2] = {nullptr, nullptr};
+  const int* ring_started[SPX_RING] = {};
+  int ring_n[SPX_RING] = {};
   std::vector<std::pair<const int*, int>> mixed_started;
-  const int* ahead_started = nullptr;
-  int ahead_n = 0;
+  unsigned* d_gate_timeouts = nullptr;
   hipStream_t mix = nullptr;
   hipEvent_t ev_join = nullptr, ev_fork = nullptr, ev_an = nullptr;
   std::mutex mix_mu;
@@ -105,6 +106,7 @@
 struct EvPair { hipEvent_t a, b; int kind; };
 extern std::atomic<bool> g_timing;
 extern std::atomic<int> g_last_concurrent;
+extern std::atomic<int> g_last_tension_stream;
 extern std::atomic<int> g_concurrent;
 extern std::atomic<bool> g_chunks_set;
 extern std::atomic<int> g_chunks;
@@ -136,15 +138,16 @@
 int walk_stream_count();
 int dev_walk_streams(int dev, hipStream_t* w, int n);
 int ring_note(spx_plan* plan, hipStream_t st);
-int ring_wait(spx_plan* plan, hipStream_t sa, const void* ws, hipStream_t st, bool* waited_prev);
-bool ring_previous_in_flight(spx_plan* plan);
+int ring_wait(spx_plan* plan, hipStream_t sa, const void* ws, hipStream_t st, unsigned* waited);
+bool ring_in_flight(spx_plan* plan, int back);
+unsigned* plan_gate_word(spx_plan* plan);
 int ring_record(spx_plan* plan, hipStream_t on, void* ws, hipStream_t st, const void* out, const void* n_out, bool detached = false);
 SpxModeEnv mode_env();
 bool device_ours_cb(void* ctx);
 struct SpxSpeedClass { int maxC; bool speedup_only, any_speed; };
 SpxSpeedClass speed_class(const spx_stream_job* jobs, int n);
 SpxModeWalk mode_walk(const SpxPlanDev& d, const SpxWalkAsk& ask);
-void spx_launch_gate(const int* started, int n_walk, unsigned max_spins, hipStream_t st);
+void spx_launch_gate(const int* started, int n_walk, unsigned max_spins, unsigned* timeouts, hipStream_t st);
 struct SpxForce { int concurrent; bool idle_start; int total_streams; hipEvent_t after_analysis; hipStream_t ahead_sa; const int** started_out;
                   bool no_exclusive;
 };
diff --git a/speedy_amd/csrc/spx_engine.hip b/speedy_amd/csrc/spx_engine.hip
--- a/speedy_amd/csrc/spx_engine.hip
+++ b/speedy_amd/csrc/spx_engine.hip
@@ -10,6 +10,7 @@
 
 std::atomic<bool> g_timing{false};
 std::atomic<int> g_last_concurrent{0};
+std::atomic<int> g_last_tension_stream{0};
 std::atomic<int> g_concurrent{1};
 std::atomic<bool> g_chunks_set{false};
 std::atomic<int> g_chunks{1};
@@ -133,32 +134,42 @@
   return d;
 }
 
-__global__ void spx_gate_kernel(const int* started, int n_walk, unsigned max_spins) {
-  if (threadIdx.x == 0) {
-    for (unsigned i = 0; i < max_spins; i++) {
-      if (__hip_atomic_load(started, __ATOMIC_RELAXED, __HIP_MEMORY_SCOPE_AGENT) >= n_walk) break;
-      __builtin_amdgcn_s_sleep(8);
-    }
-  }
-}
-void spx_launch_gate(const int* started, int n_walk, unsigned max_spins, hipStream_t st) {
-  hipLaunchKernelGGL(spx_gate_kernel, dim3(1), dim3(64), 0, st, started, n_walk, max_spins);
+__device__ static inline void spx_gate_wait(const int* started, int n_walk, unsigned max_spins, unsigned* timeouts) {
+  unsigned i = 0;
+  for (; i < max_spins; i++) {
+    if (__hip_atomic_load(started, __ATOMIC_RELAXED, __HIP_MEMORY_SCOPE_AGENT) >= n_walk) break;
+    __builtin_amdgcn_s_sleep(8);
+  }
+  if (timeouts != nullptr && spx_gate_timed_out(i, max_spins)) atomicAdd(timeouts, 1u);
+}
+__global__ void spx_gate_kernel(const int* started, int n_walk, unsigned max_spins, unsigned* timeouts) {
+  if (threadIdx.x == 0) spx_gate_wait(started, n_walk, max_spins, timeouts);
+}
+void spx_launch_gate(const int* started, int n_walk, unsigned max_spins, unsigned* timeouts, hipStream_t st) {
+  hipLaunchKernelGGL(spx_gate_kernel, dim3(1), dim3(64), 0, st, started, n_walk, max_spins, timeouts);
+}
+unsigned* plan_gate_word(spx_plan* plan) {
+  if (!plan->d_gate_timeouts) {
+    void* p = nullptr;
+    if (hipMalloc(&p, sizeof(unsigned)) != hipSuccess || hipMemset(p, 0, sizeof(unsigned)) != hipSuccess) {
+      (void)hipGetLastError();
+      if (p) (void)hipFree(p);
+      return nullptr;
+    }
+    plan->d_gate_timeouts = static_cast<unsigned*>(p);
+  }
+  return plan->d_gate_timeouts;
 }
 __global__ void __launch_bounds__(256)
 spx_stage_kernel(const unsigned* __restrict__ src, unsigned* __restrict__ dst_a, unsigned n_a, unsigned* __restrict__ dst_b,
                  unsigned n_b, unsigned* __restrict__ zero_a, unsigned nz_a, unsigned* __restrict__ zero_b, unsigned nz_b,
-                 const int* gate_started, int gate_n, unsigned gate_spins) {
+                 const int* gate_started, int gate_n, unsigned gate_spins, unsigned* gate_timeouts) {
   const unsigned stride = gridDim.x * blockDim.x, t0 = blockIdx.x * blockDim.x + threadIdx.x;
   for (unsigned i = t0; i < n_a; i += stride) dst_a[i] = src[i];
   for (unsigned i = t0; i < n_b; i += stride) dst_b[i] = src[n_a + i];
   for (unsigned i = t0; i < nz_a; i += stride) zero_a[i] = 0u;
   for (unsigned i = t0; i < nz_b; i += stride) zero_b[i] = 0u;
-  if (gate_started != nullptr && t0 == 0) {
-    for (unsigned i = 0; i < gate_spins; i++) {
-      if (__hip_atomic_load(gate_started, __ATOMIC_RELAXED, __HIP_MEMORY_SCOPE_AGENT) >= gate_n) break;
-      __builtin_amdgcn_s_sleep(8);
-    }
-  }
+  if (gate_started != nullptr && t0 == 0) spx_gate_wait(gate_started, gate_n, gate_spins, gate_timeouts);
 }
 extern "C" {
 
@@ -187,7 +198,11 @@
 #ifndef SPX_WALK_STREAMS
 #define SPX_WALK_STREAMS 3
 #endif
+#ifndef SPX_TENSION_ON_WALK
+#define SPX_TENSION_ON_WALK 0
+#endif
 int walk_stream_count() { return SPX_WALK_STREAMS; }
+extern "C" int spx_debug_tension_on_walk_enabled(void) { return SPX_TENSION_ON_WALK != 0 ? 1 : 0; }
 int dev_walk_streams(int dev, hipStream_t* w, int n) {
   static std::mutex mu;
   static hipStream_t s3[64][SPX_MAX_WALK_STREAMS];
@@ -211,21 +226,21 @@
   plan->ev_call_st[cur] = st;
   return 0;
 }
-int ring_wait(spx_plan* plan, hipStream_t sa, const void* ws, hipStream_t st, bool* waited_prev) {
+int ring_wait(spx_plan* plan, hipStream_t sa, const void* ws, hipStream_t st, unsigned* waited) {
   const int c = plan->ahead_calls % SPX_RING;
-  if (waited_prev) *waited_prev = false;
+  if (waited) *waited = 0u;
   for (int back = SPX_RING; back >= 1; back--) {
     const int j = (c + SPX_RING - back) % SPX_RING;
     if (!plan->ev_walk_valid[j]) continue;
     if (back > SPX_RING / 2 || plan->ring_ws[j] == ws || plan->ring_st[j] != st) {
       HIPCHK(hipStreamWaitEvent(sa, plan->ev_walk[j], 0));
-      if (back == 1 && waited_prev) *waited_prev = true;
-    }
-  }
-  return 0;
-}
-bool ring_previous_in_flight(spx_plan* plan) {
-  const int j = (plan->ahead_calls + SPX_RING - 1) % SPX_RING;
+      if (waited) *waited |= 1u << back;
+    }
+  }
+  return 0;
+}
+bool ring_in_flight(spx_plan* plan, int back) {
+  const int j = (plan->ahead_calls + SPX_RING - back) % SPX_RING;
   const bool f = plan->ev_walk_valid[j] && hipEventQuery(plan->ev_walk[j]) == hipErrorNotReady;
   (void)hipGetLastError();
   return f;
@@ -238,6 +253,8 @@
   plan->ev_walk_valid[c] = true;
   plan->ring_ws[c] = ws;
   plan->ring_st[c] = st;
+  plan->ring_started[c] = nullptr;
+  plan->ring_n[c] = 0;
   plan->ahead_last_out = out;
   plan->ahead_last_nout = n_out;
   plan->ahead_calls++;
@@ -314,7 +331,7 @@
 
 static int stage_tables(spx_plan* plan, const std::vector<SpxStreamDev>& sv, const std::vector<int>& order, SpxStreamDev* dstreams,
                         int* d_order, int* d_flags, unsigned n_flags, int* d_ready, unsigned n_ready, hipStream_t on, hipEvent_t* done,
-                        const int* gate_started = nullptr, int gate_n = 0, unsigned gate_spins = 0) {
+                        const int* gate_started = nullptr, int gate_n = 0, unsigned gate_spins = 0, unsigned* gate_timeouts = nullptr) {
   const size_t b_sv = sizeof(SpxStreamDev) * sv.size(), b_or = sizeof(int) * order.size();
   SpxStage& G = plan->stage[plan->stage_next];
   plan->stage_next ^= 1;
@@ -332,7 +349,7 @@
   if (b_or) memcpy(hp + b_sv, order.data(), b_or);
   hipLaunchKernelGGL(spx_stage_kernel, dim3(64), dim3(256), 0, on, reinterpret_cast<const unsigned*>(hp),
                      reinterpret_cast<unsigned*>(dstreams), (unsigned)(b_sv / 4), reinterpret_cast<unsigned*>(d_order), (unsigned)(b_or / 4),
-                     reinterpret_cast<unsigned*>(d_flags), n_flags, reinterpret_cast<unsigned*>(d_ready), n_ready, gate_started, gate_n, gate_spins);
+                     reinterpret_cast<unsigned*>(d_flags), n_flags, reinterpret_cast<unsigned*>(d_ready), n_ready, gate_started, gate_n, gate_spins, gate_timeouts);
   HIPCHK(hipEventRecord(G.done, on));
   *done = G.done;
   return 0;
@@ -416,6 +433,7 @@
   const int nch = M.nch;
   const bool concurrent = M.concurrent, ahead = M.ahead;
   const bool chunk_ahead = M.chunk_ahead && !force;
+  const bool tension_on_walk = SPX_TENSION_ON_WALK != 0 && do_a && do_w && !force && spx_tension_on_walk_stream(M, walk_stream_count());
   std::vector<SpxStreamDev> sv;
   std::vector<int> tiles;
   build_streams(d, jobs, n, nch, sv, tiles, opt.rate);
@@ -431,12 +449,13 @@
   SpxTapsDev td = taps_of(taps);
   const bool timed = g_timing.load() && do_a && do_w;
   if (do_a && do_w) g_last_concurrent.store(concurrent ? 1 : (ahead ? 2 : 0), std::memory_order_relaxed);
+  if (do_a && do_w) g_last_tension_stream.store(tension_on_walk ? 1 : 0, std::memory_order_relaxed);
   static const bool dbg_mode = getenv("SPX_DEBUG_MODE") != nullptr;
   if (dbg_mode)
     fprintf(stderr, "[spx mode] rate %d n %d maxC %d: co_resident %d doubtful %d lean %d want_concurrent %d chunks %d tiles %d -> %s%s\n",
             d.rate, n, maxC, (int)M.co_resident, (int)M.doubtful, (int)M.launch_lean, (int)M.want_concurrent, nch, tiles[0],
             concurrent ? "concurrent" : (ahead ? (M.seq_ahead ? "ahead (kernels in sequence)" : "ahead") : (chunk_ahead ? "sequence, producers ahead" : "sequence")),
-            M.walk2 ? ", walk kernels overlapping" : "");
+            M.walk2 ? (tension_on_walk ? ", walk kernels overlapping, tension kernel on the walk stream" : ", walk kernels overlapping") : "");
   hipStream_t stw = st;
   const bool detached = opt.detached && M.walk2 && !force;
   if (do_w && !force && !detached && ring_note(plan, st)) return -2;
@@ -476,18 +495,19 @@
       for (int i = 0; i < n; i++)
         if (t < cnt[i]) order.push_back(sv[i].first_tile + t);
   }
-  bool waited_prev = false;
+  unsigned waited = 0u;
   if ((ahead || chunk_ahead) && !force) {
-    if (ring_wait(plan, sa, ws, st, &waited_prev)) return -2;
+    if (ring_wait(plan, sa, ws, st, &waited)) return -2;
     if (opt.in_ready) HIPCHK(hipStreamWaitEvent(sa, static_cast<hipEvent_t>(opt.in_ready), 0));
   }
   if (!ahead && !chunk_ahead && opt.in_ready) HIPCHK(hipStreamWaitEvent(st, static_cast<hipEvent_t>(opt.in_ready), 0));
   hipEvent_t staged_ev = nullptr;
-  const bool ahead_gate = ahead && !force && plan->ahead_started != nullptr && plan->ahead_n > 0 && !waited_prev &&
-                          ring_previous_in_flight(plan);
+  const int gate_slot = (plan->ahead_calls + SPX_RING - 1) % SPX_RING;
+  const bool ahead_gate = ahead && !force && !tension_on_walk && plan->ev_walk_valid[gate_slot] && plan->ring_started[gate_slot] != nullptr &&
+                          plan->ring_n[gate_slot] > 0 && !(waited & 2u) && plan->ring_ws[gate_slot] != ws && ring_in_flight(plan, 1);
   const int rc = stage_tables(plan, sv, opt.rate ? opt.rate->table : order, dstreams, opt.rate ? reinterpret_cast<int*>(opt.rate->d_table) : d_order, d_flags, concurrent ? (unsigned)tiles[0] : 0u, d_ready,
                     (concurrent || ahead) ? (unsigned)n + 1u : 0u, (ahead || chunk_ahead) ? sa : st, &staged_ev,
-                    ahead_gate ? plan->ahead_started : nullptr, plan->ahead_n, 8000u);
+                    ahead_gate ? plan->ring_started[gate_slot] : nullptr, plan->ring_n[gate_slot], 8000u, ahead_gate ? plan_gate_word(plan) : nullptr);
   if (rc) return rc;
   if (M.trial_slot >= 0) {
     hipEvent_t& e0 = TR.ev[2 * M.trial_slot];
@@ -501,7 +521,7 @@
   for (int c = 0; c < nch; c++) {
     SpxStreamDev* dj = dstreams + (size_t)c * n;
     if (concurrent && do_w && idle_start)
-      hipLaunchKernelGGL(spx_gate_kernel, dim3(1), dim3(64), 0, sa, d_ready + n, n, 1200u);
+      hipLaunchKernelGGL(spx_gate_kernel, dim3(1), dim3(64), 0, sa, d_ready + n, n, 1200u, static_cast<unsigned*>(nullptr));
     if (do_a && tiles[c] > 0) {
       SpxTimed tm(timed, 0, sa);
       spx_launch_analysis(d, dj, n, tiles[c], in, rec, td, concurrent ? d_order : nullptr, concurrent ? d_flags : nullptr, maxC == 1, sa);
@@ -510,13 +530,14 @@
     if (sa != st) HIPCHK(hipEventRecord(plan->ev_chunk[c], sa));
     if (sa != st && !concurrent && !ahead) HIPCHK(hipStreamWaitEvent(st, plan->ev_chunk[c], 0));
     if (do_w) {
-      hipStream_t stn = concurrent ? plan->side2 : (ahead ? sa : st);
+      hipStream_t stn = concurrent ? plan->side2 : (tension_on_walk ? stw : (ahead ? sa : st));
+      if (tension_on_walk) HIPCHK(hipStreamWaitEvent(stw, plan->ev_chunk[c], 0));
       {
         SpxTimed tm(timed, 2, stn);
         spx_launch_tension(d, dj, n, states, rec, scratch, td, concurrent ? d_flags : nullptr, (concurrent || ahead) ? d_ready : nullptr, stn);
       }
-      if (concurrent || ahead) HIPCHK(hipEventRecord(plan->ev_tension, stn));
-      if (ahead) HIPCHK(hipStreamWaitEvent(stw, plan->ev_tension, 0));
+      if ((concurrent || ahead) && !tension_on_walk) HIPCHK(hipEventRecord(plan->ev_tension, stn));
+      if (ahead && !tension_on_walk) HIPCHK(hipStreamWaitEvent(stw, plan->ev_tension, 0));
       {
         SpxTimed tm(timed, 1, stw);
         const SpxWalkAsk ask = {.n_streams = n, .max_channels = maxC, .speedup_only = speedup_only, .any_speed = any_speed, .lean = M.launch_lean,
@@ -531,8 +552,9 @@
       if (M.ahead_forced && force->started_out) *force->started_out = d_ready + n;
       if (c == nch - 1 && !force) {
         if (ring_record(plan, stw, ws, st, out, n_out, detached)) return -2;
-        plan->ahead_started = (concurrent || ahead) ? d_ready + n : nullptr;
-        plan->ahead_n = n;
+        const int slot = (plan->ahead_calls + SPX_RING - 1) % SPX_RING;
+        plan->ring_started[slot] = (concurrent || ahead) ? d_ready + n : nullptr;
+        plan->ring_n[slot] = n;
         plan->mixed_started.clear();
       }
     }
diff --git a/speedy_amd/csrc/spx_mixed.hip b/speedy_amd/csrc/spx_mixed.hip
--- a/speedy_amd/csrc/spx_mixed.hip
+++ b/speedy_amd/csrc/spx_mixed.hip
@@ -178,14 +178,14 @@
   std::vector<const int*> started(n_plans, nullptr);
   if (ahead) {
     std::lock_guard<std::mutex> ring_lock(lead->mu);
-    bool waited_prev = false;
-    if (ring_wait(lead, dev_s1, ws, st, &waited_prev)) return -2;
-    const bool in_flight = !waited_prev && ring_previous_in_flight(lead);
+    unsigned waited = 0u;
+    if (ring_wait(lead, dev_s1, ws, st, &waited)) return -2;
+    const bool in_flight = !(waited & 2u) && ring_in_flight(lead, 1);
     if (in_ready) HIPCHK(hipStreamWaitEvent(dev_s1, static_cast<hipEvent_t>(in_ready), 0));
     if (upload_idx(dev_s1)) return -2;
     if (in_flight)
       for (const auto& sn : lead->mixed_started)
-        if (sn.first && sn.second > 0) spx_launch_gate(sn.first, sn.second, 8000u, dev_s1);
+        if (sn.first && sn.second > 0) spx_launch_gate(sn.first, sn.second, 8000u, plan_gate_word(lead), dev_s1);
   }
   hipEvent_t prev_an = nullptr;
   int launch_idx = 0;
@@ -234,8 +234,6 @@
   {
     std::lock_guard<std::mutex> ring_lock(lead->mu);
     if (ring_record(lead, fin, ws, st, out, n_out, walk2)) return -2;
-    lead->ahead_started = nullptr;
-    lead->ahead_n = 0;
     lead->mixed_started.clear();
     if (ahead)
       for (int g = 0; g < n_plans; g++)
diff --git a/speedy_amd/csrc/spx_mode.h b/speedy_amd/csrc/spx_mode.h
--- a/speedy_amd/csrc/spx_mode.h
+++ b/speedy_amd/csrc/spx_mode.h
@@ -182,6 +182,15 @@
   return M;
 }
 
+static inline bool spx_tension_on_walk_stream(const SpxMode& M, int walk_streams) {
+  return M.ahead && M.walk2 && !M.ahead_forced && !M.seq_ahead && !M.concurrent && !M.chunk_ahead && walk_streams >= 3;
+}
+
+#if defined(__HIPCC__)
+__host__ __device__
+#endif
+static inline bool spx_gate_timed_out(unsigned spins, unsigned bound) { return bound > 0 && spins >= bound; }
+
 struct SpxModeGroup {
   int n;
   SpxModeWalk walk;
diff --git a/speedy_amd/csrc/spx_mode_table.cpp b/speedy_amd/csrc/spx_mode_table.cpp
--- a/speedy_amd/csrc/spx_mode_table.cpp
+++ b/speedy_amd/csrc/spx_mode_table.cpp
@@ -44,8 +44,8 @@
 #undef X
       ;
 }
-int spx_mode_table_eval(const long long* q, int nq, long long* a, int na) {
-  if (nq != Q_COUNT || na != A_COUNT) return -1;
+}
+static SpxMode mode_of(const long long* q) {
   SpxModeShape S;
   SpxModeResources R;
   SpxModeEnv E;
@@ -68,7 +68,12 @@
   T.ms_seq = (float)q[Q_us_seq] / 1000.0f; T.ms_con = (float)q[Q_us_con] / 1000.0f; T.trial_key = q[Q_trial_key];
   long long ours = q[Q_device_ours];
   T.device_ours = ours_cb; T.device_ctx = &ours;
-  const SpxMode M = spx_choose_mode(S, R, E, T, trial);
+  return spx_choose_mode(S, R, E, T, trial);
+}
+extern "C" {
+int spx_mode_table_eval(const long long* q, int nq, long long* a, int na) {
+  if (nq != Q_COUNT || na != A_COUNT) return -1;
+  const SpxMode M = mode_of(q);
   a[A_lean_walk] = M.lean_walk; a[A_launch_lean] = M.launch_lean; a[A_tile_frames] = M.tile_frames; a[A_co_resident] = M.co_resident;
   a[A_doubtful] = M.doubtful; a[A_trial_slot] = M.trial_slot; a[A_want_concurrent] = M.want_concurrent; a[A_concurrent] = M.concurrent;
   a[A_ahead] = M.ahead; a[A_seq_ahead] = M.seq_ahead; a[A_ahead_forced] = M.ahead_forced; a[A_walk2] = M.walk2; a[A_nch] = M.nch;
@@ -76,6 +81,11 @@
   a[A_next_calls] = M.trial_next.calls; a[A_next_choice] = M.trial_next.choice;
   return 0;
 }
+int spx_mode_table_tension_on_walk(const long long* q, int nq, int walk_streams) {
+  if (nq != Q_COUNT) return -1;
+  return spx_tension_on_walk_stream(mode_of(q), walk_streams) ? 1 : 0;
+}
+int spx_mode_table_gate_timed_out(unsigned spins, unsigned bound) { return spx_gate_timed_out(spins, bound) ? 1 : 0; }
 int spx_mode_table_mixed_mode(const long long* groups, int n_groups, int n_total, int cu_count, long long lds_per_cu, long long tension_lds,
                               int tension_vgprs, int concurrent_enabled, int ahead_req, int guard_busy, int device_ours, long long* out4) {
   SpxModeGroup G[8];
diff --git a/speedy_amd/csrc/spx_plan.hip b/speedy_amd/csrc/spx_plan.hip
--- a/speedy_amd/csrc/spx_plan.hip
+++ b/speedy_amd/csrc/spx_plan.hip
@@ -241,6 +241,7 @@
     if (g.done) { (void)hipEventSynchronize(g.done); (void)hipEventDestroy(g.done); }
     if (g.p) (void)hipHostFree(g.p);
   }
+  if (plan->d_gate_timeouts) (void)hipFree(plan->d_gate_timeouts);
   if (plan->tables) (void)hipFree(plan->tables);
   delete plan;
 }
```

New measurement: 49520. No clear change (-0.6%).
